# zhangrengang/SubPhaser

Measured on AMD Instinct MI355X. Metric: genome Gbases/s k-mer+enrichment, wheat k=15 1Mb windows, higher is better.
Workload: dtype u32

## Files before the change

### include/subphaser_hip.h

```cpp
#ifndef SUBPHASER_HIP_H
#define SUBPHASER_HIP_H
#include <stdint.h>
#ifdef __cplusplus
extern "C" {
#endif

#define SP_OK 0
#define SP_EINVAL (-1)
#define SP_EUNSUP (-2)
#define SP_ENOMEM (-3)
#define SP_EHIP (-4)
#define SP_ENODEV (-5)
#define SP_ESTATE (-6)
#define SP_EIO (-7)

typedef struct sp_ctx sp_ctx;

int sp_version(void);
const char *sp_last_error(const sp_ctx *ctx);

int sp_ctx_create(int device, void *stream, sp_ctx **out);
int sp_ctx_destroy(sp_ctx *ctx);
int sp_sync(sp_ctx *ctx);
void *sp_stream(sp_ctx *ctx);

int sp_genome_reset(sp_ctx *ctx, int n_chrom);
int sp_genome_add(sp_ctx *ctx, int chrom, const uint8_t *ascii, int64_t len);
int sp_genome_add_device(sp_ctx *ctx, int chrom, const uint8_t *d_ascii, int64_t len);
int sp_genome_len(sp_ctx *ctx, int chrom, int64_t *len);
int sp_genome_unpack(sp_ctx *ctx, int chrom, uint8_t *ascii_out, int64_t len);

int sp_count(sp_ctx *ctx, int k, int lower_count, int engine);
int sp_count_range(sp_ctx *ctx, int k, int lower_count, int engine, int first, int last);
int sp_count_recounts(sp_ctx *ctx, int64_t *recounts);
int sp_nslots(sp_ctx *ctx, int k, int64_t *nslots);
int sp_tables_bind(sp_ctx *ctx, int chrom, void *d_table);
int sp_table_overflow(sp_ctx *ctx, int chrom, void *d_pairs, int64_t cap, int64_t *n_pairs);
int sp_table_merge(sp_ctx *ctx, void *d_dst_u8, const void *d_dst_ovf, int64_t n_dst_ovf, const void *d_src_u8,
                   const void *d_src_ovf, int64_t n_src_ovf, int64_t slot_base, int64_t n, void *d_out_ovf, int64_t cap,
                   int64_t *n_out);
int sp_table_lengths(sp_ctx *ctx, const void *d_tab_u8, const void *d_ovf, int64_t n_ovf, int64_t slot_base, int64_t n,
                     int lower_count, int64_t *sum, int64_t *n_dump);
int sp_lengths(sp_ctx *ctx, int64_t *lengths );
int sp_dump_size(sp_ctx *ctx, int chrom, int64_t *n);
int sp_dump(sp_ctx *ctx, int chrom, uint64_t *keys, uint32_t *counts, int64_t cap, int64_t *n);

int sp_filter_view(sp_ctx *ctx, int C, const void *const *d_tabs, int64_t slot_base,
                   int64_t nslots_view, const int64_t *lengths, int k, int lower_count,
                   const void *const *d_ovf, const int64_t *n_ovf);
int sp_filter(sp_ctx *ctx, int n_sets, const int32_t *set_off, const int32_t *unit_off,
              const int32_t *unit_chrom, double min_fold, int baseline, double min_freq,
              double max_freq, double ratio, int64_t *n_union, int64_t *n_rows, int64_t *n_hist);
int sp_filter_fetch(sp_ctx *ctx, uint64_t *keys, uint32_t *counts, double *freqs, uint64_t *tot,
                    int64_t cap_rows);
int sp_filter_fetch_async(sp_ctx *ctx, uint64_t *keys, uint32_t *counts, uint64_t *tot, int64_t cap_rows);
int sp_filter_fetch_wait(sp_ctx *ctx);
int sp_filter_fetch_device(sp_ctx *ctx, void *d_keys, void *d_counts, void *d_tot, int64_t cap_rows);
int sp_filter_hist(sp_ctx *ctx, uint64_t *tot, int64_t cap);

int sp_labels_set(sp_ctx *ctx, const uint64_t *keys, const uint8_t *sg, int64_t n, int n_sg);
int sp_labels_set_device(sp_ctx *ctx, const uint64_t *d_keys, const uint8_t *d_sg, int64_t n, int n_sg);
int sp_map_nslots(sp_ctx *ctx, int chrom, int64_t bin_size, int64_t chunk_size, int64_t *nslots);
int sp_map_bins(sp_ctx *ctx, int chrom, int64_t bin_size, int64_t chunk_size, int32_t *slot_counts,
                int64_t nslots, int64_t *n_mapped);
int sp_map_bins_all(sp_ctx *ctx, int64_t bin_size, int64_t chunk_size, const int64_t *slot_off,
                    int32_t *slot_counts, int64_t *n_mapped);
int sp_stack_windows(sp_ctx *ctx, int64_t bin_size, int64_t chunk_size, int64_t window_size,
                     const int64_t *slot_off, const int64_t *win_off, int64_t *win_counts);
int sp_stack_windows_dev(sp_ctx *ctx, int64_t bin_size, int64_t chunk_size, int64_t window_size,
                         const int64_t *slot_off, const int64_t *win_off, const int64_t *seg_start, void *d_win);
int sp_map_features(sp_ctx *ctx, const uint8_t *ascii, const int64_t *off, int64_t n_feat,
                    int64_t *counts);
int sp_map_intervals(sp_ctx *ctx, const int32_t *chrom, const int64_t *start, const int64_t *end, int64_t n,
                     int64_t *counts);
int sp_labels_hit(sp_ctx *ctx, int64_t *n_hit);

int sp_enrich(sp_ctx *ctx, const int64_t *counts, int64_t W, int S, double max_pval,
              double min_ratio, double *pvals, int32_t *argmin, uint8_t *sig, double *ratios);
int sp_enrich_dev(sp_ctx *ctx, const void *d_counts, int64_t W, int S, double max_pval, double min_ratio,
                  double *pvals, int32_t *argmin, uint8_t *sig, double *ratios);
int sp_stack_enrich(sp_ctx *ctx, int64_t bin_size, int64_t chunk_size, int64_t window_size, const int64_t *slot_off,
                    const int64_t *win_off, double max_pval, double min_ratio, int64_t *win_counts, double *pvals,
                    int32_t *argmin, uint8_t *sig, double *ratios);

int sp_kmer_ttest(sp_ctx *ctx, const uint32_t *counts, int64_t M, int C, const int64_t *lengths, int n_groups,
                  const int32_t *group_off, const int32_t *group_chrom, int32_t *top, int32_t *second,
                  double *pvals, double *means);

int sp_sparse_sizes(sp_ctx *ctx, int64_t *n);
int sp_sparse_sample(sp_ctx *ctx, int chrom, int64_t n_samples, uint64_t *keys, int64_t *n_out);
int sp_sparse_split(sp_ctx *ctx, int chrom, const uint64_t *splitters, int n_split, int64_t *bounds);
int sp_sparse_export(sp_ctx *ctx, int chrom, int64_t first, int64_t count, void *d_keys, void *d_counts);
int sp_sparse_view(sp_ctx *ctx, int C, const void *const *d_keys, const void *const *d_counts, const int64_t *n,
                   const int64_t *lengths, int k, int lower_count);

int sp_prof_enable(sp_ctx *ctx, int on);
int sp_prof_reset(sp_ctx *ctx);
int sp_prof_report(sp_ctx *ctx, char *buf, int64_t cap);

int sp_synth_chrom(sp_ctx *ctx, uint8_t *d_out, int64_t len, uint64_t seed, int set_id,
                   int sg_id, int n_sg, int chrom_id, int exchange);
int sp_synth_chrom_range(sp_ctx *ctx, uint8_t *d_out, int64_t len, int64_t start, int64_t n, uint64_t seed, int set_id,
                         int sg_id, int n_sg, int chrom_id, int exchange);
int sp_host_alloc(sp_ctx *ctx, int64_t bytes, void **h_ptr);
int sp_host_free(sp_ctx *ctx, void *h_ptr);
int sp_host_register(sp_ctx *ctx, void *h_ptr, int64_t bytes);
int sp_host_unregister(sp_ctx *ctx, void *h_ptr);
int sp_dev_alloc(sp_ctx *ctx, int64_t bytes, void **d_ptr);
int sp_dev_free(sp_ctx *ctx, void *d_ptr);
int sp_dev_copy_to_host(sp_ctx *ctx, void *dst, const void *d_src, int64_t bytes);
int sp_dev_copy_from_host(sp_ctx *ctx, void *d_dst, const void *src, int64_t bytes);


typedef struct sp_fasta sp_fasta;
int sp_fasta_open(const void *data, int64_t n, int threads, sp_fasta **out);
int sp_fasta_counts(const sp_fasta *h, int64_t *n_records, int64_t *n_bases);
int sp_fasta_fetch(const sp_fasta *h, int64_t *hdr_start, int64_t *hdr_end, int64_t *seq_off, void *cat);
void sp_fasta_close(sp_fasta *h);


int sp_text_kmer_matrix(const uint64_t *keys, int k, const double *freqs, int64_t M, int C, int threads, int fd,
                        int64_t *bytes);
int sp_text_sig_kmers(const uint64_t *keys, int k, const int32_t *top, const char *names, int n_names,
                      const double *pvals, const double *means, int G, int64_t M, int threads, int fd, int64_t *bytes);
int sp_text_repr(const double *x, int64_t n, char *out, int64_t *off);

#define SP_COL_STR 0
#define SP_COL_I64 1
#define SP_COL_F64 2
#define SP_COL_NAME 3
#define SP_COL_IVAL 4
typedef struct sp_text_col {
    int kind;
    int width;
    char join;
    const void *data;
    const int64_t *off;
    const char *names;
} sp_text_col;
int sp_text_table(const sp_text_col *cols, int n_cols, int64_t M, int threads, int fd, int64_t *bytes);

#ifdef __cplusplus
}
#endif
#endif
```

### subphaser_amd/_native.py

```python
import ctypes as C
import json
import os

import numpy as np

_HERE = os.path.dirname(os.path.abspath(__file__))
LIB_PATH = os.environ.get("SUBPHASER_HIP_LIB") or os.path.join(_HERE, "lib", "libsubphaser_hip.so")

SP_OK, SP_EINVAL, SP_EUNSUP, SP_ENOMEM, SP_EHIP, SP_ENODEV, SP_ESTATE, SP_EIO = 0, -1, -2, -3, -4, -5, -6, -7

SYMBOLS = [
    "sp_version", "sp_last_error", "sp_ctx_create", "sp_ctx_destroy", "sp_sync", "sp_stream",
    "sp_genome_reset", "sp_genome_add", "sp_genome_add_device", "sp_genome_len", "sp_genome_unpack",
    "sp_count", "sp_count_range", "sp_count_recounts", "sp_nslots", "sp_tables_bind", "sp_table_overflow", "sp_table_merge", "sp_table_lengths", "sp_lengths", "sp_dump_size", "sp_dump",
    "sp_filter_view", "sp_filter", "sp_filter_fetch", "sp_filter_fetch_async", "sp_filter_fetch_wait", "sp_filter_fetch_device", "sp_filter_hist",
    "sp_labels_set", "sp_labels_set_device", "sp_map_nslots", "sp_map_bins", "sp_map_bins_all", "sp_stack_windows", "sp_stack_windows_dev", "sp_stack_enrich", "sp_map_features", "sp_map_intervals", "sp_labels_hit",
    "sp_enrich", "sp_enrich_dev", "sp_kmer_ttest",
    "sp_sparse_sizes", "sp_sparse_sample", "sp_sparse_split", "sp_sparse_export", "sp_sparse_view",
    "sp_prof_enable", "sp_prof_reset", "sp_prof_report",
    "sp_synth_chrom", "sp_synth_chrom_range", "sp_host_alloc", "sp_host_free", "sp_host_register", "sp_host_unregister", "sp_dev_alloc", "sp_dev_free", "sp_dev_copy_to_host", "sp_dev_copy_from_host",
    "sp_fasta_open", "sp_fasta_counts", "sp_fasta_fetch", "sp_fasta_close",
    "sp_text_kmer_matrix", "sp_text_sig_kmers", "sp_text_repr", "sp_text_table",
]


def csrc_fingerprint():
    import glob
    import hashlib
    h = hashlib.sha256()
    files = sorted(glob.glob(os.path.join(_HERE, "csrc", "*.hip")) + glob.glob(os.path.join(_HERE, "csrc", "*.h")))
    for f in files:
        h.update(os.path.basename(f).encode())
        h.update(open(f, "rb").read())
    return h.hexdigest()[:16]


class NativeError(RuntimeError):
    """HIP/runtime failure inside libsubphaser_hip.so."""


_lib = None


def load():
    global _lib
    if _lib is not None:
        return _lib
    if not os.path.exists(LIB_PATH):
        raise NativeError(
            "libsubphaser_hip.so is not built (%s). Run `python -c 'import __graft_entry__ as g; g.build()'` "
            "or `make -C subphaser_amd/csrc`. There is no CPU fallback." % LIB_PATH)
    L = C.CDLL(LIB_PATH)
    vp, i64, i32, dbl, ci = C.c_void_p, C.c_int64, C.c_int32, C.c_double, C.c_int
    P = C.POINTER
    L.sp_version.restype = ci
    L.sp_last_error.restype = C.c_char_p
    L.sp_last_error.argtypes = [vp]
    L.sp_ctx_create.argtypes = [ci, vp, P(vp)]
    L.sp_ctx_destroy.argtypes = [vp]
    L.sp_sync.argtypes = [vp]
    L.sp_stream.restype = vp
    L.sp_stream.argtypes = [vp]
    L.sp_genome_reset.argtypes = [vp, ci]
    L.sp_genome_add.argtypes = [vp, ci, vp, i64]
    L.sp_genome_add_device.argtypes = [vp, ci, vp, i64]
    L.sp_genome_len.argtypes = [vp, ci, P(i64)]
    L.sp_genome_unpack.argtypes = [vp, ci, vp, i64]
    L.sp_count.argtypes = [vp, ci, ci, ci]
    L.sp_count_range.argtypes = [vp, ci, ci, ci, ci, ci]
    L.sp_nslots.argtypes = [vp, ci, P(i64)]
    L.sp_count_recounts.argtypes = [vp, P(i64)]
    L.sp_tables_bind.argtypes = [vp, ci, vp]
    L.sp_table_overflow.argtypes = [vp, ci, vp, i64, P(i64)]
    L.sp_table_merge.argtypes = [vp, vp, vp, i64, vp, vp, i64, i64, i64, vp, i64, P(i64)]
    L.sp_table_lengths.argtypes = [vp, vp, vp, i64, i64, i64, ci, P(i64), P(i64)]
    L.sp_filter_view.argtypes = [vp, ci, vp, i64, i64, vp, ci, ci, vp, vp]
    L.sp_lengths.argtypes = [vp, vp]
    L.sp_dump_size.argtypes = [vp, ci, P(i64)]
    L.sp_dump.argtypes = [vp, ci, vp, vp, i64, P(i64)]
    L.sp_filter.argtypes = [vp, ci, vp, vp, vp, dbl, ci, dbl, dbl, dbl, P(i64), P(i64), P(i64)]
    L.sp_filter_fetch.argtypes = [vp, vp, vp, vp, vp, i64]
    L.sp_filter_fetch_device.argtypes = [vp, vp, vp, vp, i64]
    L.sp_filter_fetch_async.argtypes = [vp, vp, vp, vp, i64]
    L.sp_filter_fetch_wait.argtypes = [vp]
    L.sp_filter_hist.argtypes = [vp, vp, i64]
    L.sp_labels_set.argtypes = [vp, vp, vp, i64, ci]
    L.sp_labels_set_device.argtypes = [vp, vp, vp, i64, ci]
    L.sp_map_nslots.argtypes = [vp, ci, i64, i64, P(i64)]
    L.sp_map_bins.argtypes = [vp, ci, i64, i64, vp, i64, P(i64)]
    L.sp_map_bins_all.argtypes = [vp, i64, i64, vp, vp, vp]
    L.sp_stack_windows.argtypes = [vp, i64, i64, i64, vp, vp, vp]
    L.sp_stack_windows_dev.argtypes = [vp, i64, i64, i64, vp, vp, vp, vp]
    L.sp_stack_enrich.argtypes = [vp, i64, i64, i64, vp, vp, dbl, dbl, vp, vp, vp, vp, vp]
    L.sp_map_features.argtypes = [vp, vp, vp, i64, vp]
    L.sp_map_intervals.argtypes = [vp, vp, vp, vp, i64, vp]
    L.sp_host_alloc.argtypes = [vp, i64, P(vp)]
    L.sp_host_free.argtypes = [vp, vp]
    L.sp_labels_hit.argtypes = [vp, P(i64)]
    L.sp_enrich.argtypes = [vp, vp, i64, ci, dbl, dbl, vp, vp, vp, vp]
    L.sp_enrich_dev.argtypes = [vp, vp, i64, ci, dbl, dbl, vp, vp, vp, vp]
    L.sp_kmer_ttest.argtypes = [vp, vp, i64, ci, vp, ci, vp, vp, vp, vp, vp, vp]
    L.sp_sparse_sizes.argtypes = [vp, vp]
    L.sp_sparse_sample.argtypes = [vp, ci, i64, vp, P(i64)]
    L.sp_sparse_split.argtypes = [vp, ci, vp, ci, vp]
    L.sp_sparse_export.argtypes = [vp, ci, i64, i64, vp, vp]
    L.sp_sparse_view.argtypes = [vp, ci, vp, vp, vp, vp, ci, ci]
    L.sp_prof_enable.argtypes = [vp, ci]
    L.sp_prof_reset.argtypes = [vp]
    L.sp_prof_report.argtypes = [vp, C.c_char_p, i64]
    L.sp_synth_chrom.argtypes = [vp, vp, i64, C.c_uint64, ci, ci, ci, ci, ci]
    L.sp_synth_chrom_range.argtypes = [vp, vp, i64, i64, i64, C.c_uint64, ci, ci, ci, ci, ci]
    L.sp_dev_alloc.argtypes = [vp, i64, P(vp)]
    L.sp_dev_free.argtypes = [vp, vp]
    L.sp_dev_copy_to_host.argtypes = [vp, vp, vp, i64]
    L.sp_host_register.argtypes = [vp, vp, i64]
    L.sp_host_unregister.argtypes = [vp, vp]
    L.sp_dev_copy_from_host.argtypes = [vp, vp, vp, i64]
    L.sp_fasta_open.argtypes = [vp, i64, ci, P(vp)]
    L.sp_fasta_counts.argtypes = [vp, P(i64), P(i64)]
    L.sp_fasta_fetch.argtypes = [vp, vp, vp, vp, vp]
    L.sp_fasta_close.argtypes = [vp]
    L.sp_fasta_close.restype = None
    L.sp_text_kmer_matrix.argtypes = [vp, ci, vp, i64, ci, ci, ci, P(i64)]
    L.sp_text_sig_kmers.argtypes = [vp, ci, vp, C.c_char_p, ci, vp, vp, ci, i64, ci, ci, P(i64)]
    L.sp_text_repr.argtypes = [vp, i64, vp, vp]
    L.sp_text_table.argtypes = [vp, ci, i64, ci, ci, P(i64)]
    for name in SYMBOLS:
        if name not in ("sp_last_error", "sp_stream", "sp_fasta_close"):
            getattr(L, name).restype = ci
    _lib = L
    return L


def _p(a):
    return a.ctypes.data_as(C.c_void_p) if a is not None else None


def fasta_scan(data, threads=None, out=None):
    L = load()
    data = np.frombuffer(data, np.uint8) if isinstance(data, (bytes, bytearray, memoryview)) else data
    if data.dtype != np.uint8 or not data.flags.c_contiguous:
        data = np.ascontiguousarray(data, np.uint8)
    n = int(data.size)
    if threads is None:
        threads = min(32, len(os.sched_getaffinity(0)))
    h = C.c_void_p()
    rc = L.sp_fasta_open(C.c_void_p(data.ctypes.data) if n else None, n, int(threads), C.byref(h))
    if rc == SP_ENOMEM:
        raise MemoryError("sp_fasta_open")
    if rc:
        raise ValueError("sp_fasta_open: bad arguments")
    try:
        nr, nb = C.c_int64(), C.c_int64()
        L.sp_fasta_counts(h, C.byref(nr), C.byref(nb))
        nr, nb = nr.value, nb.value
        hs, he, off = np.empty(nr, np.int64), np.empty(nr, np.int64), np.empty(nr + 1, np.int64)
        cat = out(nb) if out is not None else np.empty(nb, np.uint8)
        if L.sp_fasta_fetch(h, _p(hs), _p(he), _p(off), _p(cat) if nb else None):
            raise ValueError("sp_fasta_fetch: bad arguments")
    finally:
        L.sp_fasta_close(h)
    ids = []
    for a, b in zip(hs.tolist(), he.tolist()):
        t = bytes(data[a:b]).split()
        ids.append(t[0].decode() if t else "")
    return ids, cat, off


def _fd_of(fout):
    try:
        fd = fout.fileno()
        fout.flush()
        return fd
    except Exception:
        return None


def _text_threads():
    return min(64, len(os.sched_getaffinity(0)))


def _text_fail(name, rc):
    msg = load().sp_last_error(None).decode(errors="replace")
    if rc == SP_ENOMEM:
        raise MemoryError("%s: %s" % (name, msg or "out of memory"))
    raise OSError("%s failed (%d): %s" % (name, rc, msg))


def text_kmer_matrix(fout, keys, k, freqs):
    fd = _fd_of(fout)
    if fd is None:
        return False
    keys = np.ascontiguousarray(keys, np.uint64)
    freqs = np.ascontiguousarray(freqs, np.float64)
    M, Cn = freqs.shape
    rc = load().sp_text_kmer_matrix(_p(keys), int(k), _p(freqs), M, Cn, _text_threads(), fd, None)
    if rc:
        _text_fail("sp_text_kmer_matrix", rc)
    return True


def text_sig_kmers(fout, keys, k, top, names, pvals, means):
    fd = _fd_of(fout)
    if fd is None:
        return False
    keys = np.ascontiguousarray(keys, np.uint64)
    top = np.ascontiguousarray(top, np.int32)
    pvals = np.ascontiguousarray(pvals, np.float64)
    means = np.ascontiguousarray(means, np.float64)
    blob = b"".join(n.encode() + b"\0" for n in names)
    rc = load().sp_text_sig_kmers(_p(keys), int(k), _p(top), blob, len(names), _p(pvals), _p(means), means.shape[1],
                                  len(keys), _text_threads(), fd, None)
    if rc:
        _text_fail("sp_text_sig_kmers", rc)
    return True


class _TextCol(C.Structure):
    _fields_ = [("kind", C.c_int), ("width", C.c_int), ("join", C.c_char), ("data", C.c_void_p),
                ("off", C.c_void_p), ("names", C.c_void_p)]


def str_blob(strings):
    enc = [s.encode() for s in strings]
    off = np.zeros(len(enc) + 1, np.int64)
    if enc:
        np.cumsum(np.fromiter((len(e) for e in enc), np.int64, len(enc)), out=off[1:])
    return np.frombuffer(b"".join(enc) or b"\0", np.uint8), off


def write_chunks(fout, n_rows, format_rows, chunk=50000):
    for lo in range(0, max(0, n_rows), chunk):
        fout.write(format_rows(lo, min(lo + chunk, n_rows)))


def text_table(fout, n_rows, cols):
    fd = _fd_of(fout)
    if fd is None:
        return False
    arr = (_TextCol * len(cols))()
    keep = []
    for c, col in zip(arr, cols):
        kind = col[0]
        if kind == "str":
            blob, off = np.ascontiguousarray(col[1], np.uint8), np.ascontiguousarray(col[2], np.int64)
            assert off.size == n_rows + 1
            c.kind, c.width, c.join, c.data, c.off = 0, 1, b"\t", blob.ctypes.data, off.ctypes.data
            keep += [blob, off]
        elif kind in ("i64", "f64"):
            a = np.ascontiguousarray(col[1], np.int64 if kind == "i64" else np.float64).reshape(n_rows, -1)
            c.kind, c.width, c.join, c.data = (1 if kind == "i64" else 2), max(1, a.shape[1]), col[2].encode(), a.ctypes.data
            keep.append(a)
        elif kind == "ival":
            a = np.ascontiguousarray(col[1], np.int64).reshape(n_rows, 3)
            blob, off = str_blob(col[2])
            c.kind, c.width, c.join, c.data, c.off, c.names = 4, len(col[2]), b"\t", a.ctypes.data, off.ctypes.data, blob.ctypes.data
            keep += [a, blob, off]
        elif kind == "name":
            idx = np.ascontiguousarray(col[1], np.int32)
            blob, off = str_blob(col[2])
            assert idx.size == n_rows
            c.kind, c.width, c.join, c.data, c.off, c.names = 3, len(col[2]), b"\t", idx.ctypes.data, off.ctypes.data, blob.ctypes.data
            keep += [idx, blob, off]
        else:
            raise ValueError(kind)
    rc = load().sp_text_table(arr, len(cols), int(n_rows), _text_threads(), fd, None)
    if rc:
        _text_fail("sp_text_table", rc)
    return True


def text_repr(x):
    x = np.ascontiguousarray(x, np.float64)
    out = np.empty(max(1, x.size * 40), np.uint8)
    off = np.empty(x.size + 1, np.int64)
    load().sp_text_repr(_p(x), x.size, _p(out), _p(off))
    b = out.tobytes()
    return [b[off[i]:off[i + 1]].decode() for i in range(x.size)]


def as_ascii(seq):
    if isinstance(seq, str):
        seq = seq.encode()
    if isinstance(seq, (bytes, bytearray, memoryview)):
        return np.frombuffer(seq, dtype=np.uint8)
    return np.ascontiguousarray(seq, dtype=np.uint8)


class Context:

    def __init__(self, device=0, stream=None):
        self.L = load()
        h = C.c_void_p()
        rc = self.L.sp_ctx_create(int(device), C.c_void_p(stream) if stream else None, C.byref(h))
        if rc != SP_OK:
            raise NativeError("sp_ctx_create failed (%d): %s" % (rc, self.L.sp_last_error(None).decode()))
        self.h = h
        self.n_chrom = 0
        self.k = None
        self._pinned = {}

    def _ck(self, rc):
        if rc == SP_OK:
            return
        msg = self.L.sp_last_error(self.h).decode()
        if rc in (SP_ESTATE, SP_EINVAL, SP_EUNSUP):
            raise ValueError(msg)
        if rc == SP_ENOMEM:
            raise MemoryError(msg)
        raise NativeError("libsubphaser_hip error %d: %s" % (rc, msg))

    def close(self):
        if getattr(self, "h", None):
            for d_keys, d_sg in getattr(self, "_label_copies", {}).values():
                self.L.sp_dev_free(self.h, C.c_void_p(d_keys))
                self.L.sp_dev_free(self.h, C.c_void_p(d_sg))
            self._label_copies = {}
            for ptr, _ in self._pinned.values():
                self.L.sp_host_free(self.h, C.c_void_p(ptr))
            self._pinned = {}
            self.L.sp_ctx_destroy(self.h)
            self.h = None

    def pinned_empty(self, tag, shape, dtype):
        dtype = np.dtype(dtype)
        n = int(np.prod(shape)) * dtype.itemsize
        ptr, cap = self._pinned.get(tag, (None, 0))
        if n > cap or ptr is None:
            if ptr:
                self.L.sp_host_free(self.h, C.c_void_p(ptr))
            p = C.c_void_p()
            want = n + n // 8 + 4096
            self._ck(self.L.sp_host_alloc(self.h, want, C.byref(p)))
            ptr, cap = p.value, want
            self._pinned[tag] = (ptr, cap)
        buf = (C.c_uint8 * max(n, 1)).from_address(ptr)
        return np.frombuffer(buf, dtype=dtype, count=int(np.prod(shape))).reshape(shape)

    def __del__(self):
        try:
            self.close()
        except Exception:
            pass

    def __enter__(self):
        return self

    def __exit__(self, *a):
        self.close()

    def sync(self):
        self._ck(self.L.sp_sync(self.h))

    @property
    def stream(self):
        return self.L.sp_stream(self.h)

    def genome_reset(self, n_chrom):
        self._ck(self.L.sp_genome_reset(self.h, int(n_chrom)))
        self.n_chrom = int(n_chrom)

    def genome_add(self, chrom, seq):
        a = as_ascii(seq)
        self._ck(self.L.sp_genome_add(self.h, int(chrom), _p(a), a.size))

    def genome_add_device(self, chrom, d_ptr, length):
        self._ck(self.L.sp_genome_add_device(self.h, int(chrom), C.c_void_p(int(d_ptr)), int(length)))

    def genome_len(self, chrom):
        n = C.c_int64()
        self._ck(self.L.sp_genome_len(self.h, int(chrom), C.byref(n)))
        return n.value

    def genome_unpack(self, chrom):
        n = self.genome_len(chrom)
        out = np.empty(n, np.uint8)
        self._ck(self.L.sp_genome_unpack(self.h, int(chrom), _p(out), n))
        return out

    def count(self, k, lower_count=3, engine=0):
        self._ck(self.L.sp_count(self.h, int(k), int(lower_count), int(engine)))
        self.k = int(k)

    def count_range(self, k, lower_count, engine, first, last):
        self._ck(self.L.sp_count_range(self.h, int(k), int(lower_count), int(engine), int(first), int(last)))
        self.k = int(k)

    def count_recounts(self):
        n = C.c_int64()
        self._ck(self.L.sp_count_recounts(self.h, C.byref(n)))
        return n.value

    def nslots(self, k):
        n = C.c_int64()
        self._ck(self.L.sp_nslots(self.h, int(k), C.byref(n)))
        return n.value

    def tables_bind(self, chrom, d_ptr):
        self._ck(self.L.sp_tables_bind(self.h, int(chrom), C.c_void_p(int(d_ptr)) if d_ptr else None))

    def table_overflow(self, chrom, d_pairs=None, cap=0):
        n = C.c_int64()
        self._ck(self.L.sp_table_overflow(self.h, int(chrom), C.c_void_p(int(d_pairs)) if d_pairs else None, int(cap),
                                          C.byref(n)))
        return n.value

    def table_merge(self, d_dst, d_dst_ovf, n_dst_ovf, d_src, d_src_ovf, n_src_ovf, slot_base, n, d_out_ovf, cap):
        m = C.c_int64()
        self._ck(self.L.sp_table_merge(self.h, C.c_void_p(int(d_dst)), C.c_void_p(int(d_dst_ovf)) if n_dst_ovf else None,
                                       int(n_dst_ovf), C.c_void_p(int(d_src)),
                                       C.c_void_p(int(d_src_ovf)) if n_src_ovf else None, int(n_src_ovf), int(slot_base),
                                       int(n), C.c_void_p(int(d_out_ovf)) if cap else None, int(cap), C.byref(m)))
        return m.value

    def table_lengths(self, d_tab, d_ovf, n_ovf, slot_base, n, lower_count):
        a, b = C.c_int64(), C.c_int64()
        self._ck(self.L.sp_table_lengths(self.h, C.c_void_p(int(d_tab)), C.c_void_p(int(d_ovf)) if n_ovf else None,
                                         int(n_ovf), int(slot_base), int(n), int(lower_count), C.byref(a), C.byref(b)))
        return a.value, b.value

    def filter_view(self, d_ptrs, slot_base, nslots_view, lengths, k, lower_count, d_ovf=None, n_ovf=None):
        if d_ptrs is None:
            self._ck(self.L.sp_filter_view(self.h, 0, None, 0, 0, None, 0, 0, None, None))
            self._view_C = None
            return
        arr = (C.c_void_p * len(d_ptrs))(*[int(p) for p in d_ptrs])
        lengths = np.ascontiguousarray(lengths, np.int64)
        oarr, narr = None, None
        if d_ovf is not None:
            oarr = (C.c_void_p * len(d_ptrs))(*[int(p) if p else None for p in d_ovf])
            narr = _p(np.ascontiguousarray(n_ovf, np.int64))
        self._ck(self.L.sp_filter_view(self.h, len(d_ptrs), arr, int(slot_base), int(nslots_view), _p(lengths),
                                       int(k), int(lower_count), oarr, narr))
        self._view_C = len(d_ptrs)
        self.k = int(k)

    def sparse_sizes(self):
        out = np.zeros(self.n_chrom, np.int64)
        if self.n_chrom:
            self._ck(self.L.sp_sparse_sizes(self.h, _p(out)))
        return out

    def sparse_sample(self, chrom, n_samples):
        out = np.empty(int(n_samples), np.uint64)
        n = C.c_int64()
        self._ck(self.L.sp_sparse_sample(self.h, int(chrom), int(n_samples), _p(out), C.byref(n)))
        return out[:n.value]

    def sparse_split(self, chrom, splitters):
        sp = np.ascontiguousarray(splitters, np.uint64)
        bounds = np.zeros(sp.size + 2, np.int64)
        self._ck(self.L.sp_sparse_split(self.h, int(chrom), _p(sp), int(sp.size), _p(bounds)))
        return bounds

    def sparse_export(self, chrom, first, count, d_keys, d_counts):
        v = lambda p: C.c_void_p(int(p)) if p else None
        self._ck(self.L.sp_sparse_export(self.h, int(chrom), int(first), int(count), v(d_keys), v(d_counts)))

    def sparse_view(self, d_keys, d_counts, n, lengths, k, lower_count):
        if d_keys is None:
            self._ck(self.L.sp_sparse_view(self.h, 0, None, None, None, None, 0, 0))
            self._view_C = None
            return
        ka = (C.c_void_p * len(d_keys))(*[int(p) for p in d_keys])
        ca = (C.c_void_p * len(d_counts))(*[int(p) for p in d_counts])
        n = np.ascontiguousarray(n, np.int64)
        lengths = np.ascontiguousarray(lengths, np.int64)
        self._ck(self.L.sp_sparse_view(self.h, len(d_keys), ka, ca, _p(n), _p(lengths), int(k), int(lower_count)))
        self._view_C = len(d_keys)
        self.k = int(k)

    def lengths(self):
        out = np.zeros(self.n_chrom, np.int64)
        self._ck(self.L.sp_lengths(self.h, _p(out)))
        return out

    def dump_size(self, chrom):
        n = C.c_int64()
        self._ck(self.L.sp_dump_size(self.h, int(chrom), C.byref(n)))
        return n.value

    def dump(self, chrom, sort=True):
        n = C.c_int64()
        self._ck(self.L.sp_dump_size(self.h, int(chrom), C.byref(n)))
        keys = np.empty(n.value, np.uint64)
        cnts = np.empty(n.value, np.uint32)
        self._ck(self.L.sp_dump(self.h, int(chrom), _p(keys), _p(cnts), n.value, C.byref(n)))
        if sort and keys.size:
            o = np.argsort(keys, kind="stable")
            keys, cnts = keys[o], cnts[o]
        return keys, cnts

    def filter(self, set_off, unit_off, unit_chrom, min_fold, baseline, min_freq, max_freq, ratio):
        set_off = np.ascontiguousarray(set_off, np.int32)
        unit_off = np.ascontiguousarray(unit_off, np.int32)
        unit_chrom = np.ascontiguousarray(unit_chrom, np.int32)
        nu, nr, nh = C.c_int64(), C.c_int64(), C.c_int64()
        self._ck(self.L.sp_filter(self.h, len(set_off) - 1, _p(set_off), _p(unit_off), _p(unit_chrom),
                                  float(min_fold), int(baseline), float(min_freq), float(max_freq),
                                  float(ratio), C.byref(nu), C.byref(nr), C.byref(nh)))
        return nu.value, nr.value, nh.value

    def filter_fetch(self, n_rows, want_freqs=True, sort=True, pinned=False):
        Cn = getattr(self, "_view_C", None) or self.n_chrom
        if pinned and not sort:
            keys = self.pinned_empty("ff_keys", (n_rows,), np.uint64)
            counts = self.pinned_empty("ff_counts", (n_rows, Cn), np.uint32)
            tot = self.pinned_empty("ff_tot", (n_rows,), np.uint64)
            freqs = self.pinned_empty("ff_freqs", (n_rows, Cn), np.float64) if want_freqs else None
        else:
            keys = np.empty(n_rows, np.uint64)
            counts = np.empty((n_rows, Cn), np.uint32)
            tot = np.empty(n_rows, np.uint64)
            freqs = np.empty((n_rows, Cn), np.float64) if want_freqs else None
        self._ck(self.L.sp_filter_fetch(self.h, _p(keys), _p(counts), _p(freqs), _p(tot), n_rows))
        if sort and n_rows:
            o = np.argsort(keys, kind="stable")
            keys, counts, tot = keys[o], counts[o], tot[o]
            if freqs is not None:
                freqs = freqs[o]
        return keys, counts, freqs, tot

    def filter_fetch_async(self, n_rows):
        Cn = getattr(self, "_view_C", None) or self.n_chrom
        keys = self.pinned_empty("ff_keys", (n_rows,), np.uint64)
        counts = self.pinned_empty("ff_counts", (n_rows, Cn), np.uint32)
        tot = self.pinned_empty("ff_tot", (n_rows,), np.uint64)
        self._ck(self.L.sp_filter_fetch_async(self.h, _p(keys), _p(counts), _p(tot), n_rows))
        return keys, counts, tot

    def filter_fetch_async_ptr(self, h_keys, h_counts, n_rows):
        tot = self.pinned_empty("ff_tot", (max(int(n_rows), 1),), np.uint64)
        self._ck(self.L.sp_filter_fetch_async(self.h, C.c_void_p(int(h_keys)), C.c_void_p(int(h_counts)), _p(tot), int(n_rows)))

    def filter_fetch_wait(self):
        self._ck(self.L.sp_filter_fetch_wait(self.h))

    def filter_fetch_device(self, d_keys, d_counts, d_tot, n_rows):
        v = lambda p: C.c_void_p(int(p)) if p else None
        self._ck(self.L.sp_filter_fetch_device(self.h, v(d_keys), v(d_counts), v(d_tot), int(n_rows)))

    def filter_hist(self, n_hist):
        tot = np.empty(n_hist, np.uint64)
        self._ck(self.L.sp_filter_hist(self.h, _p(tot), n_hist))
        return tot

    def labels_set(self, keys, sg, n_sg):
        keys = np.ascontiguousarray(keys, np.uint64)
        sg = np.ascontiguousarray(sg, np.uint8)
        assert keys.size == sg.size
        self._ck(self.L.sp_labels_set(self.h, _p(keys), _p(sg), keys.size, int(n_sg)))
        self.n_sg = int(n_sg)

    def labels_set_device(self, d_keys, d_sg, n, n_sg):
        self._ck(self.L.sp_labels_set_device(self.h, C.c_void_p(int(d_keys)), C.c_void_p(int(d_sg)), int(n), int(n_sg)))
        self.n_sg = int(n_sg)

    def labels_set_from(self, labels, n_sg):
        if hasattr(labels, "on_device"):
            d_keys, d_sg = labels.on_device(self)
            self.labels_set_device(d_keys, d_sg, len(labels.keys), n_sg)
        else:
            self.labels_set(labels.keys, labels.sg_idx, n_sg)

    def map_nslots(self, chrom, bin_size, chunk_size):
        n = C.c_int64()
        self._ck(self.L.sp_map_nslots(self.h, int(chrom), int(bin_size), int(chunk_size), C.byref(n)))
        return n.value

    def map_bins(self, chrom, bin_size=10000, chunk_size=10_000_000):
        ns = self.map_nslots(chrom, bin_size, chunk_size)
        out = np.empty((ns, self.n_sg), np.int32)
        n = C.c_int64()
        self._ck(self.L.sp_map_bins(self.h, int(chrom), int(bin_size), int(chunk_size), _p(out), ns,
                                    C.byref(n)))
        return out, n.value

    def map_bins_all(self, bin_size=10000, chunk_size=10_000_000):
        off = np.zeros(self.n_chrom + 1, np.int64)
        for i in range(self.n_chrom):
            off[i + 1] = off[i] + self.map_nslots(i, bin_size, chunk_size)
        out = self.pinned_empty("map_all", (int(off[-1]), self.n_sg), np.int32)
        nm = np.zeros(self.n_chrom, np.int64)
        self._ck(self.L.sp_map_bins_all(self.h, int(bin_size), int(chunk_size), _p(off), _p(out), _p(nm)))
        self.last_map = (out, off)
        return [out[off[i]:off[i + 1]] for i in range(self.n_chrom)], nm

    def stack_windows(self, bin_size, chunk_size, window_size, lengths):
        out, off = self.last_map
        woff = np.zeros(self.n_chrom + 1, np.int64)
        for i, n in enumerate(lengths):
            woff[i + 1] = woff[i] + (int(n) + int(window_size) - 1) // int(window_size) + 1
        win = self.pinned_empty("win_all", (int(woff[-1]), self.n_sg), np.int64)
        self._ck(self.L.sp_stack_windows(self.h, int(bin_size), int(chunk_size), int(window_size), _p(off),
                                         _p(woff), _p(win)))
        return win, woff

    def stack_windows_dev(self, bin_size, chunk_size, window_size, win_off, seg_start, d_win):
        out, off = self.last_map
        win_off = np.ascontiguousarray(win_off, np.int64)
        seg = np.ascontiguousarray(seg_start, np.int64) if seg_start is not None else None
        self._ck(self.L.sp_stack_windows_dev(self.h, int(bin_size), int(chunk_size), int(window_size), _p(off),
                                             _p(win_off), _p(seg) if seg is not None else None, C.c_void_p(int(d_win))))

    def stack_enrich(self, bin_size, chunk_size, window_size, lengths, max_pval=0.05, min_ratio=0.5):
        out, off = self.last_map
        woff = np.zeros(self.n_chrom + 1, np.int64)
        for i, n in enumerate(lengths):
            woff[i + 1] = woff[i] + (int(n) + int(window_size) - 1) // int(window_size) + 1
        W, S = int(woff[-1]), self.n_sg
        win = self.pinned_empty("win_all", (W, S), np.int64)
        pvals = self.pinned_empty("enr_p", (W, S), np.float64)
        ratios = self.pinned_empty("enr_q", (W, S), np.float64)
        argmin = self.pinned_empty("enr_a", (W,), np.int32)
        sig = self.pinned_empty("enr_s", (W,), np.uint8)
        self._ck(self.L.sp_stack_enrich(self.h, int(bin_size), int(chunk_size), int(window_size), _p(off), _p(woff),
                                        float(max_pval), float(min_ratio), _p(win), _p(pvals), _p(argmin), _p(sig),
                                        _p(ratios)))
        return win, woff, pvals, argmin, sig, ratios

    def enrich_dev(self, d_counts, W, S, max_pval=0.05, min_ratio=0.5):
        pvals = np.empty((W, S), np.float64)
        ratios = np.empty((W, S), np.float64)
        argmin = np.empty(W, np.int32)
        sig = np.empty(W, np.uint8)
        self._ck(self.L.sp_enrich_dev(self.h, C.c_void_p(int(d_counts)), int(W), int(S), float(max_pval),
                                      float(min_ratio), _p(pvals), _p(argmin), _p(sig), _p(ratios)))
        return pvals, argmin, sig.astype(bool), ratios

    def map_features(self, seqs):
        arrs = [as_ascii(s) for s in seqs]
        off = np.zeros(len(arrs) + 1, np.int64)
        for i, a in enumerate(arrs):
            off[i + 1] = off[i] + a.size
        cat = np.concatenate(arrs) if arrs else np.empty(0, np.uint8)
        cat = np.ascontiguousarray(cat)
        out = np.zeros((len(arrs), self.n_sg), np.int64)
        self._ck(self.L.sp_map_features(self.h, _p(cat), _p(off), len(arrs), _p(out)))
        return out

    def map_features_cat(self, cat, off):
        cat = np.ascontiguousarray(cat, np.uint8)
        off = np.ascontiguousarray(off, np.int64)
        n = off.size - 1
        out = np.zeros((n, self.n_sg), np.int64)
        self._ck(self.L.sp_map_features(self.h, _p(cat), _p(off), n, _p(out)))
        return out

    def map_intervals(self, chrom, start, end):
        chrom = np.ascontiguousarray(chrom, np.int32)
        start = np.ascontiguousarray(start, np.int64)
        end = np.ascontiguousarray(end, np.int64)
        assert chrom.size == start.size == end.size
        out = np.zeros((chrom.size, self.n_sg), np.int64)
        self._ck(self.L.sp_map_intervals(self.h, _p(chrom), _p(start), _p(end), chrom.size, _p(out)))
        return out

    def labels_hit(self):
        n = C.c_int64()
        self._ck(self.L.sp_labels_hit(self.h, C.byref(n)))
        return n.value

    def enrich(self, counts, max_pval=0.05, min_ratio=0.5):
        counts = np.ascontiguousarray(counts, np.int64)
        if counts.ndim != 2:
            raise ValueError("counts must be W x S")
        W, S = counts.shape
        pvals = np.empty((W, S), np.float64)
        ratios = np.empty((W, S), np.float64)
        argmin = np.empty(W, np.int32)
        sig = np.empty(W, np.uint8)
        self._ck(self.L.sp_enrich(self.h, _p(counts), W, S, float(max_pval), float(min_ratio), _p(pvals),
                                  _p(argmin), _p(sig), _p(ratios)))
        return pvals, argmin, sig.astype(bool), ratios

    def kmer_ttest(self, counts, lengths, groups):
        if isinstance(counts, tuple):
            d_ptr, M, Cn = counts
            cptr = C.c_void_p(int(d_ptr))
        else:
            counts = np.ascontiguousarray(counts, np.uint32)
            M, Cn = counts.shape
            cptr = _p(counts)
        lengths = np.ascontiguousarray(lengths, np.int64)
        goff = np.zeros(len(groups) + 1, np.int32)
        goff[1:] = np.cumsum([len(g) for g in groups])
        gch = np.ascontiguousarray(np.concatenate([np.asarray(g, np.int32) for g in groups]), np.int32)
        top, second = np.empty(M, np.int32), np.empty(M, np.int32)
        pvals, means = np.empty(M, np.float64), np.empty((M, len(groups)), np.float64)
        self._ck(self.L.sp_kmer_ttest(self.h, cptr, M, Cn, _p(lengths), len(groups), _p(goff), _p(gch),
                                      _p(top), _p(second), _p(pvals), _p(means)))
        return top, second, pvals, means

    def stage_rows(self, counts):
        counts = np.ascontiguousarray(counts, np.uint32)
        old = getattr(self, "_staged_rows", None)
        if old:
            self.dev_free(old)
            self._staged_rows = None
        if counts.size == 0:
            return None
        self._staged_rows = self.dev_alloc(counts.nbytes)
        self.host_to_dev(self._staged_rows, counts)
        return (self._staged_rows, counts.shape[0], counts.shape[1])

    def release_rows(self):
        old = getattr(self, "_staged_rows", None)
        if old:
            self.dev_free(old)
            self._staged_rows = None

    def prof_enable(self, on=True):
        self._ck(self.L.sp_prof_enable(self.h, 1 if on else 0))

    def prof_reset(self):
        self._ck(self.L.sp_prof_reset(self.h))

    def prof_report(self):
        buf = C.create_string_buffer(1 << 16)
        self._ck(self.L.sp_prof_report(self.h, buf, len(buf)))
        return json.loads(buf.value.decode())

    def dev_alloc(self, nbytes):
        p = C.c_void_p()
        self._ck(self.L.sp_dev_alloc(self.h, int(nbytes), C.byref(p)))
        return p.value

    def dev_free(self, ptr):
        self._ck(self.L.sp_dev_free(self.h, C.c_void_p(ptr)))

    def dev_to_host(self, ptr, nbytes, offset=0):
        out = np.empty(nbytes, np.uint8)
        self._ck(self.L.sp_dev_copy_to_host(self.h, _p(out), C.c_void_p(ptr + offset), int(nbytes)))
        return out

    def host_register(self, h_ptr, nbytes):
        self._ck(self.L.sp_host_register(self.h, C.c_void_p(int(h_ptr)), int(nbytes)))

    def host_unregister(self, h_ptr):
        self._ck(self.L.sp_host_unregister(self.h, C.c_void_p(int(h_ptr))))

    def dev_to_host_ptr(self, h_ptr, d_ptr, nbytes):
        if nbytes:
            self._ck(self.L.sp_dev_copy_to_host(self.h, C.c_void_p(int(h_ptr)), C.c_void_p(int(d_ptr)), int(nbytes)))

    def host_to_dev(self, ptr, arr, offset=0):
        arr = np.ascontiguousarray(arr)
        self._ck(self.L.sp_dev_copy_from_host(self.h, C.c_void_p(ptr + offset), _p(arr), int(arr.nbytes)))

    def synth_chrom_range(self, d_ptr, length, start, n, seed, set_id, sg_id, n_sg, chrom_id, exchange=0):
        self._ck(self.L.sp_synth_chrom_range(self.h, C.c_void_p(d_ptr), int(length), int(start), int(n), int(seed),
                                             int(set_id), int(sg_id), int(n_sg), int(chrom_id), int(exchange)))

    def synth_chrom(self, d_ptr, length, seed, set_id, sg_id, n_sg, chrom_id, exchange=0):
        self._ck(self.L.sp_synth_chrom(self.h, C.c_void_p(d_ptr), int(length), int(seed), int(set_id),
                                       int(sg_id), int(n_sg), int(chrom_id), int(exchange)))
```

### subphaser_amd/csrc/sp_common.h

```cpp
#pragma once
#include <hip/hip_runtime.h>
#include <stdint.h>
#include <stdio.h>
#include <string.h>

#include <map>
#include <string>
#include <vector>

#include "../../include/subphaser_hip.h"

#define SP_WAVE 64

struct sp_chrom {
    bool tab_external = false;
    int64_t len = 0;
    int64_t nw = 0;
    int64_t cap_mw = 0;
    uint32_t *d_pk = nullptr;
    uint32_t *d_pm = nullptr;
    uint32_t *d_nm = nullptr;
    uint8_t *d_tab = nullptr;
    uint2 *d_ovf = nullptr;
    int64_t n_ovf = 0, cap_ovf = 0;
    uint32_t *d_ovf_idx = nullptr;
    int64_t ovf_idx_n = 0, ovf_idx_cap = 0;
    int64_t length_sum = 0;
    int64_t n_dump = 0;
    hipEvent_t ev_packed = nullptr;
};
#define SP_PAD_WORDS 8
#define SP_LIST_MAXC 1024
#define SP_TABLE_LDS (140 * 1024)
#define SP_TABLE_MIN_TILE 256
#define SP_TABLE_MAXC (SP_TABLE_LDS / SP_TABLE_MIN_TILE)
#ifndef SP_DERIVE_PM
#define SP_DERIVE_PM 1
#endif

struct sp_buf {
    void *p = nullptr;
    int64_t cap = 0;
};

template <typename T>
struct sp_tmp {
    T *p = nullptr;
    sp_tmp() = default;
    sp_tmp(const sp_tmp &) = delete;
    sp_tmp &operator=(const sp_tmp &) = delete;
    ~sp_tmp() {
        if (p) hipFree(p);
    }
    hipError_t alloc(size_t n_elems) { return hipMalloc((void **)&p, (n_elems ? n_elems : 1) * sizeof(T)); }
    operator T *() const { return p; }
};

struct sp_sparse_chrom {
    uint64_t *d_keys = nullptr;
    uint32_t *d_cnts = nullptr;
    int64_t n = 0, cap = 0, length_sum = 0;
};

struct sp_tabref {
    const uint8_t *tab;
    const uint2 *ovf;
    int64_t n_ovf;
    const uint32_t *ovf_idx = nullptr;
};

struct sp_prof_entry {
    std::string name;
    hipEvent_t e0, e1;
};

struct sp_ctx {
    int device = 0;
    hipStream_t stream = nullptr;
    hipStream_t copy_stream = nullptr;
    hipEvent_t copy_event = nullptr;
    bool own_stream = false;
    int n_cu = 256;
    std::string err;
    std::vector<sp_chrom> chroms;
    int k = 0;
    int lower = 0;
    int64_t nslots = 0;
    bool counted = false;
    int64_t c2_recounts = 0;
    bool fv_on = false;
    std::vector<sp_tabref> fv_tabs;
    std::vector<int64_t> fv_lengths;
    int64_t fv_slot_base = 0, fv_nslots = 0;
    bool sv_on = false;
    std::vector<const uint64_t *> sv_keys;
    std::vector<const uint32_t *> sv_cnts;
    std::vector<int64_t> sv_n;
    bool filtered = false;
    int64_t n_union = 0, n_rows = 0, n_hist = 0;
    uint32_t *d_flag_row = nullptr;
    uint32_t *d_flag_hist = nullptr;
    uint64_t *d_blk_row = nullptr;
    uint64_t *d_blk_hist = nullptr;
    int64_t n_fblocks = 0;
    uint8_t *d_label = nullptr;
    sp_buf b_ptab, b_labkeys;
    int ptab_k = 0;
    int64_t ptab_n = 0;
    unsigned long long *h_lflags = nullptr;
    sp_buf b_lflags;
    int64_t bloom_last_n = -1;
    int bloom_last_bits = 0, bloom_last_k = 0;
    sp_buf b_ctab, b_covf;
    int ct_bb = 0;
    uint32_t ct_ovf_mask = 0;
    int sq_bb = 0;
    uint64_t sq_ovf_mask = 0;
    int map_engine = 0;
    bool labels_ready = false;
    uint32_t *d_bloom = nullptr;
    int bloom_bits = 0;
    int n_sg = 0;
    int64_t n_labels = 0;
    void *d_scratch = nullptr;
    int64_t scratch_bytes = 0;
    void *d_ws2 = nullptr;
    int64_t ws2_bytes = 0;
    sp_buf b_cntlen;
    sp_buf b_tab32, b_ovfw;
    struct lane_t {
        hipStream_t stream = nullptr;
        hipEvent_t done = nullptr;
        void *d_ws2 = nullptr;
        int64_t ws2_bytes = 0;
        sp_buf b_ovfw;
        void *h_desc = nullptr;
        int64_t h_desc_cap = 0;
        sp_buf b_sp_a, b_sp_b, b_sp_c, b_sp_tmp, b_s3_small;
        hipEvent_t ev_a = nullptr, ev_b = nullptr;
    };
#define SP_MAX_LANES 7
    lane_t lanes[SP_MAX_LANES];
    lane_t *lane = nullptr;
    void *h_desc = nullptr;
    int64_t h_desc_cap = 0;
    hipEvent_t lane_go = nullptr;
    bool sparse_mode = false;
    bool list_mode = false;
    std::vector<sp_sparse_chrom> sparse;
    sp_buf b_sp_a, b_sp_b, b_sp_c, b_sp_tmp, b_sf_keys, b_sf_counts, b_sf_tot, b_sf_hist, b_s3_small, b_slots;
    unsigned long long *h_s3 = nullptr;
    hipEvent_t s3_ev[2] = {nullptr, nullptr};
    int64_t sf_n = 0;
    uint64_t *d_hkeys = nullptr;
    int64_t hcap = 0;
    sp_buf b_tt;
    sp_buf b_wtab, b_enr;
    sp_buf b_fq;
    sp_buf b_fflat;
    sp_buf b_map, b_mapdesc, b_ival, b_emit, b_fpar, b_win;
    bool map_all_valid = false;
    bool prof = false;
    std::vector<sp_prof_entry> prof_pending;
    std::map<std::string, std::pair<int64_t, double>> prof_acc;
};

extern thread_local std::string g_sp_err;

int sp_fail(sp_ctx *ctx, int code, const char *fmt, ...);
int sp_scratch(sp_ctx *ctx, int64_t bytes, void **out);
struct sp_ctx;
int sp_buf_ensure(sp_ctx *ctx, sp_buf &b, int64_t bytes);
void sp_buf_free(sp_buf &b);
void sp_prof_begin(sp_ctx *ctx, const char *name);
void sp_prof_end(sp_ctx *ctx);
void sp_prof_flush(sp_ctx *ctx);

#define SP_HIP(ctx, call)                                                                  \
    do {                                                                                   \
        hipError_t e__ = (call);                                                           \
        if (e__ != hipSuccess)                                                             \
            return sp_fail(ctx, e__ == hipErrorOutOfMemory ? SP_ENOMEM : SP_EHIP,          \
                           "%s failed: %s (%s:%d)", #call, hipGetErrorString(e__), __FILE__, \
                           __LINE__);                                                      \
    } while (0)

#define SP_LAUNCH(ctx, name, kernel, grid, block, shmem, ...)                       \
    do {                                                                            \
        sp_prof_begin(ctx, name);                                                   \
        hipLaunchKernelGGL(kernel, grid, block, shmem, (ctx)->stream, __VA_ARGS__); \
        sp_prof_end(ctx);                                                           \
        SP_HIP(ctx, hipGetLastError());                                             \
    } while (0)

struct sp_kparams {
    int k;
    int odd;
    uint64_t kmask;
    int rcshift;
};

__host__ __device__ inline sp_kparams sp_make_kparams(int k) {
    sp_kparams p;
    p.k = k;
    p.odd = k & 1;
    p.kmask = (k == 32) ? ~0ULL : ((1ULL << (2 * k)) - 1ULL);
    p.rcshift = 2 * (k - 1);
    return p;
}

__host__ __device__ inline int64_t sp_dense_slots(int k) {
    return (k & 1) ? (1LL << (2 * k - 1)) : (1LL << (2 * k));
}

__host__ __device__ inline uint64_t sp_slot_of(uint64_t fwd, uint64_t rc, const sp_kparams &p) {
    if (p.odd) {
        uint64_t rep = ((fwd >> p.k) & 1ULL) ? rc : fwd;
        uint64_t lowmask = (1ULL << p.k) - 1ULL;
        return (rep & lowmask) | ((rep >> (p.k + 1)) << p.k);
    }
    return fwd < rc ? fwd : rc;
}

__host__ __device__ inline uint64_t sp_revcomp(uint64_t x, int k) {
    x = ~x;
    x = ((x >> 2) & 0x3333333333333333ULL) | ((x & 0x3333333333333333ULL) << 2);
    x = ((x >> 4) & 0x0F0F0F0F0F0F0F0FULL) | ((x & 0x0F0F0F0F0F0F0F0FULL) << 4);
    x = ((x >> 8) & 0x00FF00FF00FF00FFULL) | ((x & 0x00FF00FF00FF00FFULL) << 8);
    x = ((x >> 16) & 0x0000FFFF0000FFFFULL) | ((x & 0x0000FFFF0000FFFFULL) << 16);
    x = (x >> 32) | (x << 32);
    return x >> (64 - 2 * k);
}

__host__ __device__ inline uint64_t sp_key_of_slot(uint64_t slot, const sp_kparams &p) {
    if (p.odd) {
        uint64_t lowmask = (1ULL << p.k) - 1ULL;
        uint64_t rep = (slot & lowmask) | ((slot >> p.k) << (p.k + 1));
        uint64_t r = sp_revcomp(rep, p.k);
        return rep < r ? rep : r;
    }
    return slot;
}

__host__ __device__ inline uint64_t sp_slot_of_key(uint64_t key, const sp_kparams &p) {
    return sp_slot_of(key, sp_revcomp(key, p.k), p);
}
```

### subphaser_amd/csrc/sp_ctx.hip

```cpp
#include <stdarg.h>

#include "sp_common.h"

thread_local std::string g_sp_err;

int sp_fail(sp_ctx *ctx, int code, const char *fmt, ...) {
    char buf[1024];
    va_list ap;
    va_start(ap, fmt);
    vsnprintf(buf, sizeof buf, fmt, ap);
    va_end(ap);
    if (ctx) ctx->err = buf;
    g_sp_err = buf;
    return code;
}

int sp_scratch(sp_ctx *ctx, int64_t bytes, void **out) {
    if (bytes > ctx->scratch_bytes) {
        if (ctx->d_scratch) {
            SP_HIP(ctx, hipStreamSynchronize(ctx->stream));
            SP_HIP(ctx, hipFree(ctx->d_scratch));
            ctx->d_scratch = nullptr;
            ctx->scratch_bytes = 0;
        }
        SP_HIP(ctx, hipMalloc(&ctx->d_scratch, (size_t)bytes));
        ctx->scratch_bytes = bytes;
    }
    *out = ctx->d_scratch;
    return SP_OK;
}

int sp_buf_ensure(sp_ctx *ctx, sp_buf &b, int64_t bytes) {
    if (bytes <= b.cap) return SP_OK;
    if (b.p) {
        SP_HIP(ctx, hipStreamSynchronize(ctx->stream));
        SP_HIP(ctx, hipFree(b.p));
        b.p = nullptr;
        b.cap = 0;
    }
    int64_t want = bytes + bytes / 8 + 4096;
    SP_HIP(ctx, hipMalloc(&b.p, (size_t)want));
    b.cap = want;
    return SP_OK;
}
void sp_buf_free(sp_buf &b) {
    if (b.p) hipFree(b.p);
    b.p = nullptr;
    b.cap = 0;
}

void sp_prof_begin(sp_ctx *ctx, const char *name) {
    if (!ctx->prof) return;
    sp_prof_entry e;
    e.name = name;
    hipEventCreate(&e.e0);
    hipEventCreate(&e.e1);
    hipEventRecord(e.e0, ctx->stream);
    ctx->prof_pending.push_back(e);
}
void sp_prof_end(sp_ctx *ctx) {
    if (!ctx->prof) return;
    hipEventRecord(ctx->prof_pending.back().e1, ctx->stream);
}
void sp_prof_flush(sp_ctx *ctx) {
    if (ctx->prof_pending.empty()) return;
    hipStreamSynchronize(ctx->stream);
    for (auto &e : ctx->prof_pending) {
        float ms = 0.f;
        hipEventElapsedTime(&ms, e.e0, e.e1);
        auto &acc = ctx->prof_acc[e.name];
        acc.first += 1;
        acc.second += ms;
        hipEventDestroy(e.e0);
        hipEventDestroy(e.e1);
    }
    ctx->prof_pending.clear();
}

void sp_sparse_release(sp_ctx *ctx);

extern "C" {

int sp_version(void) { return 100; }

const char *sp_last_error(const sp_ctx *ctx) { return ctx ? ctx->err.c_str() : g_sp_err.c_str(); }

int sp_ctx_create(int device, void *stream, sp_ctx **out) {
    if (!out) return sp_fail(nullptr, SP_EINVAL, "sp_ctx_create: out is NULL");
    int n = 0;
    if (hipGetDeviceCount(&n) != hipSuccess || n <= 0)
        return sp_fail(nullptr, SP_ENODEV, "no HIP device visible (libsubphaser_hip needs an MI355X)");
    if (device < 0 || device >= n)
        return sp_fail(nullptr, SP_EINVAL, "device %d out of range (0..%d)", device, n - 1);
    sp_ctx *ctx = new sp_ctx();
    ctx->device = device;
    SP_HIP(ctx, hipSetDevice(device));
    hipDeviceProp_t prop;
    SP_HIP(ctx, hipGetDeviceProperties(&prop, device));
    ctx->n_cu = prop.multiProcessorCount;
    if (stream) {
        ctx->stream = (hipStream_t)stream;
    } else {
        SP_HIP(ctx, hipStreamCreateWithFlags(&ctx->stream, hipStreamNonBlocking));
        ctx->own_stream = true;
    }
    *out = ctx;
    return SP_OK;
}

static void free_chrom(sp_chrom &c) {
    if (c.d_pk) hipFree(c.d_pk);
    if (c.d_nm) hipFree(c.d_nm);
    if (c.d_tab && !c.tab_external) hipFree(c.d_tab);
    if (c.d_ovf) hipFree(c.d_ovf);
    if (c.d_ovf_idx) hipFree(c.d_ovf_idx);
    c.d_ovf_idx = nullptr;
    c.ovf_idx_n = c.ovf_idx_cap = 0;
    if (c.ev_packed) hipEventDestroy(c.ev_packed);
    c = sp_chrom();
}

static void free_filter(sp_ctx *ctx) {
    if (ctx->d_flag_row) hipFree(ctx->d_flag_row);
    if (ctx->d_flag_hist) hipFree(ctx->d_flag_hist);
    if (ctx->d_blk_row) hipFree(ctx->d_blk_row);
    if (ctx->d_blk_hist) hipFree(ctx->d_blk_hist);
    ctx->d_flag_row = ctx->d_flag_hist = nullptr;
    ctx->d_blk_row = ctx->d_blk_hist = nullptr;
    ctx->filtered = false;
}

int sp_ctx_destroy(sp_ctx *ctx) {
    if (!ctx) return SP_OK;
    hipSetDevice(ctx->device);
    hipStreamSynchronize(ctx->stream);
    sp_prof_flush(ctx);
    for (auto &c : ctx->chroms) free_chrom(c);
    free_filter(ctx);
    sp_sparse_release(ctx);
    if (ctx->d_label) hipFree(ctx->d_label);
    if (ctx->d_bloom) hipFree(ctx->d_bloom);
    if (ctx->d_scratch) hipFree(ctx->d_scratch);
    if (ctx->d_ws2) hipFree(ctx->d_ws2);
    for (auto &ln : ctx->lanes) {
        if (ln.d_ws2) hipFree(ln.d_ws2);
        sp_buf_free(ln.b_ovfw);
        if (ln.h_desc) hipHostFree(ln.h_desc);
        sp_buf_free(ln.b_sp_a);
        sp_buf_free(ln.b_sp_b);
        sp_buf_free(ln.b_sp_c);
        sp_buf_free(ln.b_sp_tmp);
        sp_buf_free(ln.b_s3_small);
        if (ln.ev_a) hipEventDestroy(ln.ev_a);
        if (ln.ev_b) hipEventDestroy(ln.ev_b);
        if (ln.done) hipEventDestroy(ln.done);
        if (ln.stream) hipStreamDestroy(ln.stream);
    }
    if (ctx->lane_go) hipEventDestroy(ctx->lane_go);
    if (ctx->h_s3) hipHostFree(ctx->h_s3);
    if (ctx->h_desc) hipHostFree(ctx->h_desc);
    for (auto &e : ctx->s3_ev)
        if (e) hipEventDestroy(e);
    sp_buf_free(ctx->b_map);
    sp_buf_free(ctx->b_mapdesc);
    sp_buf_free(ctx->b_ival);
    sp_buf_free(ctx->b_ptab);
    sp_buf_free(ctx->b_lflags);
    if (ctx->h_lflags) hipHostFree(ctx->h_lflags);
    sp_buf_free(ctx->b_cntlen);
    sp_buf_free(ctx->b_ctab);
    sp_buf_free(ctx->b_covf);
    sp_buf_free(ctx->b_tab32);
    sp_buf_free(ctx->b_ovfw);
    sp_buf_free(ctx->b_labkeys);
    sp_buf_free(ctx->b_emit);
    sp_buf_free(ctx->b_slots);
    sp_buf_free(ctx->b_fpar);
    sp_buf_free(ctx->b_fflat);
    sp_buf_free(ctx->b_fq);
    sp_buf_free(ctx->b_wtab);
    sp_buf_free(ctx->b_enr);
    sp_buf_free(ctx->b_tt);
    sp_buf_free(ctx->b_win);
    if (ctx->copy_stream) {
        hipStreamSynchronize(ctx->copy_stream);
        hipStreamDestroy(ctx->copy_stream);
        hipEventDestroy(ctx->copy_event);
    }
    if (ctx->own_stream) hipStreamDestroy(ctx->stream);
    delete ctx;
    return SP_OK;
}

int sp_sync(sp_ctx *ctx) {
    SP_HIP(ctx, hipStreamSynchronize(ctx->stream));
    return SP_OK;
}

void *sp_stream(sp_ctx *ctx) { return (void *)ctx->stream; }

int sp_genome_reset(sp_ctx *ctx, int n_chrom) {
    if (!ctx || n_chrom < 0) return sp_fail(ctx, SP_EINVAL, "sp_genome_reset: bad arguments");
    SP_HIP(ctx, hipSetDevice(ctx->device));
    SP_HIP(ctx, hipStreamSynchronize(ctx->stream));
    if ((size_t)n_chrom == ctx->chroms.size()) {
        for (auto &c : ctx->chroms) {
            c.len = 0;
            c.nw = 0;
            c.length_sum = 0;
            c.n_dump = 0;
            c.n_ovf = 0;
            c.ovf_idx_n = 0;
        }
    } else {
        for (auto &c : ctx->chroms) free_chrom(c);
        ctx->chroms.assign((size_t)n_chrom, sp_chrom());
    }
    ctx->counted = false;
    ctx->filtered = false;
    return SP_OK;
}
}

__device__ __forceinline__ void pack_byte(uint32_t b, uint32_t &code, uint32_t &inv) {
    uint32_t u = b & 0xDFu;
    code = ((b >> 1) ^ (b >> 2)) & 3u;
    inv = !(u == 'A' || u == 'C' || u == 'G' || u == 'T');
}

__device__ __forceinline__ void pack_word4(uint32_t w, uint32_t &c8, uint32_t &inv4) {
    uint32_t t = ((w >> 1) ^ (w >> 2)) & 0x03030303u;
    const uint32_t letters = __builtin_amdgcn_perm(0u, 0x54474341u, t);
    const uint32_t x = letters ^ (w & 0xDFDFDFDFu);
    const uint32_t f = ((((x & 0x7F7F7F7Fu) + 0x7F7F7F7Fu) | x) & 0x80808080u) >> 7;
    t &= ~(f * 3u);
    t |= t >> 6;
    t |= t >> 12;
    c8 = t & 0xFFu;
    inv4 = ((f * 0x00204081u) >> 21) & 0xFu;
}
__device__ __forceinline__ uint32_t pack_msb_first(uint32_t w) {
    const uint32_t r = __brev(w);
    return ((r & 0x55555555u) << 1) | ((r >> 1) & 0x55555555u);
}

__global__ void __launch_bounds__(256)
k0_pack(const uint8_t *__restrict__ ascii, int64_t len, uint32_t *__restrict__ pk, uint32_t *__restrict__ pm,
        uint32_t *__restrict__ nm, int64_t n_mask_words) {
    int64_t t = (int64_t)blockIdx.x * blockDim.x + threadIdx.x;
    int64_t stride = (int64_t)gridDim.x * blockDim.x;
    const bool aligned = (((uintptr_t)ascii) & 15) == 0;
    for (; t < n_mask_words; t += stride) {
        int64_t base = t * 32;
        uint32_t w0 = 0, w1 = 0, m = 0, r0 = 0, r1 = 0;
        if (base + 32 <= len && aligned) {
            const uint4 *p = reinterpret_cast<const uint4 *>(ascii + base);
            uint4 a = p[0], b = p[1];
            uint32_t v[8] = {a.x, a.y, a.z, a.w, b.x, b.y, b.z, b.w};
#pragma unroll
            for (int q = 0; q < 8; q++) {
                uint32_t c8, inv4;
                pack_word4(v[q], c8, inv4);
                if (q < 4) w0 |= c8 << (8 * q);
                else w1 |= c8 << (8 * (q - 4));
                m |= inv4 << (4 * q);
            }
            r0 = pack_msb_first(w0);
            r1 = pack_msb_first(w1);
        } else {
            for (int i = 0; i < 32; i++) {
                uint32_t c = 0, iv = 1;
                if (base + i < len) pack_byte(ascii[base + i], c, iv);
                if (iv) c = 0;
                if (i < 16) { w0 |= c << (2 * i); r0 |= c << (30 - 2 * i); }
                else { w1 |= c << (2 * (i - 16)); r1 |= c << (30 - 2 * (i - 16)); }
                m |= iv << i;
            }
        }
        *reinterpret_cast<uint2 *>(pk + 2 * t) = make_uint2(w0, w1);
#if !SP_DERIVE_PM
        *reinterpret_cast<uint2 *>(pm + 2 * t) = make_uint2(r0, r1);
#else
        (void)r0; (void)r1; (void)pm;
#endif
        nm[t] = m;
    }
}

__global__ void __launch_bounds__(256)
k0_unpack(const uint32_t *__restrict__ pk, const uint32_t *__restrict__ nm, int64_t len,
          uint8_t *__restrict__ out) {
    int64_t i = (int64_t)blockIdx.x * blockDim.x + threadIdx.x;
    int64_t stride = (int64_t)gridDim.x * blockDim.x;
    for (; i < len; i += stride) {
        uint32_t c = (pk[i >> 4] >> (2 * (i & 15))) & 3u;
        uint32_t iv = (nm[i >> 5] >> (i & 31)) & 1u;
        out[i] = iv ? 'N' : "ACGT"[c];
    }
}

static int genome_add_impl(sp_ctx *ctx, int chrom, const uint8_t *d_ascii, int64_t len) {
    sp_chrom &c = ctx->chroms[(size_t)chrom];
    c.len = len;
    c.length_sum = 0;
    c.n_dump = 0;
    int64_t nmw = (len + 31) / 32 + SP_PAD_WORDS;
    c.nw = (len + 15) / 16;
    if (nmw > c.cap_mw) {
        if (c.d_pk) hipFree(c.d_pk);
        if (c.d_nm) hipFree(c.d_nm);
        c.d_pk = c.d_pm = c.d_nm = nullptr;
        c.cap_mw = 0;
#if SP_DERIVE_PM
        SP_HIP(ctx, hipMalloc(&c.d_pk, (size_t)(2 * nmw) * sizeof(uint32_t)));
        c.d_pm = c.d_pk;
#else
        SP_HIP(ctx, hipMalloc(&c.d_pk, (size_t)(4 * nmw) * sizeof(uint32_t)));
        c.d_pm = c.d_pk + 2 * nmw;
#endif
        SP_HIP(ctx, hipMalloc(&c.d_nm, (size_t)nmw * sizeof(uint32_t)));
        c.cap_mw = nmw;
    }
    int64_t blocks = (nmw + 255) / 256;
    if (blocks > 8LL * ctx->n_cu * 8) blocks = 8LL * ctx->n_cu * 8;
    if (blocks < 1) blocks = 1;
    SP_LAUNCH(ctx, "k0_pack", k0_pack, dim3((unsigned)blocks), dim3(256), 0, d_ascii, len, c.d_pk,
              c.d_pm, c.d_nm, nmw);
    if (!c.ev_packed) SP_HIP(ctx, hipEventCreateWithFlags(&c.ev_packed, hipEventDisableTiming));
    SP_HIP(ctx, hipEventRecord(c.ev_packed, ctx->stream));
    ctx->counted = false;
    return SP_OK;
}

extern "C" {

int sp_genome_add_device(sp_ctx *ctx, int chrom, const uint8_t *d_ascii, int64_t len) {
    if (!ctx || chrom < 0 || chrom >= (int)ctx->chroms.size() || len < 0 || (!d_ascii && len > 0))
        return sp_fail(ctx, SP_EINVAL, "sp_genome_add_device: bad arguments (chrom=%d len=%lld)", chrom,
                       (long long)len);
    SP_HIP(ctx, hipSetDevice(ctx->device));
    return genome_add_impl(ctx, chrom, d_ascii, len);
}

int sp_genome_add(sp_ctx *ctx, int chrom, const uint8_t *ascii, int64_t len) {
    if (!ctx || chrom < 0 || chrom >= (int)ctx->chroms.size() || len < 0 || (!ascii && len > 0))
        return sp_fail(ctx, SP_EINVAL, "sp_genome_add: bad arguments (chrom=%d len=%lld)", chrom,
                       (long long)len);
    SP_HIP(ctx, hipSetDevice(ctx->device));
    uint8_t *d = nullptr;
    SP_HIP(ctx, hipMalloc(&d, (size_t)(len > 0 ? len : 1)));
    hipError_t e = hipMemcpyAsync(d, ascii, (size_t)len, hipMemcpyHostToDevice, ctx->stream);
    int rc = SP_OK;
    if (e != hipSuccess) rc = sp_fail(ctx, SP_EHIP, "H2D copy failed: %s", hipGetErrorString(e));
    if (rc == SP_OK) rc = genome_add_impl(ctx, chrom, d, len);
    hipStreamSynchronize(ctx->stream);
    hipFree(d);
    return rc;
}

int sp_genome_len(sp_ctx *ctx, int chrom, int64_t *len) {
    if (!ctx || !len || chrom < 0 || chrom >= (int)ctx->chroms.size())
        return sp_fail(ctx, SP_EINVAL, "sp_genome_len: bad arguments");
    *len = ctx->chroms[(size_t)chrom].len;
    return SP_OK;
}

int sp_genome_unpack(sp_ctx *ctx, int chrom, uint8_t *ascii_out, int64_t len) {
    if (!ctx || chrom < 0 || chrom >= (int)ctx->chroms.size() || !ascii_out)
        return sp_fail(ctx, SP_EINVAL, "sp_genome_unpack: bad arguments");
    sp_chrom &c = ctx->chroms[(size_t)chrom];
    if (len != c.len) return sp_fail(ctx, SP_EINVAL, "sp_genome_unpack: len mismatch");
    if (len == 0) return SP_OK;
    SP_HIP(ctx, hipSetDevice(ctx->device));
    uint8_t *d = nullptr;
    SP_HIP(ctx, hipMalloc(&d, (size_t)len));
    int64_t blocks = (len + 255) / 256;
    if (blocks > 65536) blocks = 65536;
    SP_LAUNCH(ctx, "k0_unpack", k0_unpack, dim3((unsigned)blocks), dim3(256), 0, c.d_pk, c.d_nm, len, d);
    SP_HIP(ctx, hipMemcpyAsync(ascii_out, d, (size_t)len, hipMemcpyDeviceToHost, ctx->stream));
    SP_HIP(ctx, hipStreamSynchronize(ctx->stream));
    hipFree(d);
    return SP_OK;
}

int sp_prof_enable(sp_ctx *ctx, int on) {
    if (!ctx) return SP_EINVAL;
    if (!on) sp_prof_flush(ctx);
    ctx->prof = on != 0;
    return SP_OK;
}
int sp_prof_reset(sp_ctx *ctx) {
    if (!ctx) return SP_EINVAL;
    sp_prof_flush(ctx);
    ctx->prof_acc.clear();
    return SP_OK;
}
int sp_prof_report(sp_ctx *ctx, char *buf, int64_t cap) {
    if (!ctx || !buf || cap < 3) return SP_EINVAL;
    sp_prof_flush(ctx);
    std::string s = "{";
    bool first = true;
    for (auto &kv : ctx->prof_acc) {
        char tmp[256];
        snprintf(tmp, sizeof tmp, "%s\"%s\": {\"calls\": %lld, \"ms\": %.6f}", first ? "" : ", ",
                 kv.first.c_str(), (long long)kv.second.first, kv.second.second);
        s += tmp;
        first = false;
    }
    s += "}";
    if ((int64_t)s.size() + 1 > cap) return sp_fail(ctx, SP_EINVAL, "sp_prof_report: buffer too small");
    memcpy(buf, s.c_str(), s.size() + 1);
    return SP_OK;
}

int sp_host_alloc(sp_ctx *ctx, int64_t bytes, void **h_ptr) {
    if (!ctx || !h_ptr || bytes < 0) return sp_fail(ctx, SP_EINVAL, "sp_host_alloc: bad arguments");
    SP_HIP(ctx, hipSetDevice(ctx->device));
    SP_HIP(ctx, hipHostMalloc(h_ptr, (size_t)(bytes > 0 ? bytes : 1), hipHostMallocDefault));
    return SP_OK;
}
int sp_host_free(sp_ctx *ctx, void *h_ptr) {
    if (!ctx) return SP_EINVAL;
    SP_HIP(ctx, hipHostFree(h_ptr));
    return SP_OK;
}
int sp_host_register(sp_ctx *ctx, void *h_ptr, int64_t bytes) {
    if (!ctx || !h_ptr || bytes <= 0) return sp_fail(ctx, SP_EINVAL, "sp_host_register: bad arguments");
    SP_HIP(ctx, hipSetDevice(ctx->device));
    SP_HIP(ctx, hipHostRegister(h_ptr, (size_t)bytes, hipHostRegisterPortable));
    return SP_OK;
}
int sp_host_unregister(sp_ctx *ctx, void *h_ptr) {
    if (!ctx || !h_ptr) return SP_EINVAL;
    SP_HIP(ctx, hipHostUnregister(h_ptr));
    return SP_OK;
}
int sp_dev_alloc(sp_ctx *ctx, int64_t bytes, void **d_ptr) {
    if (!ctx || !d_ptr || bytes < 0) return sp_fail(ctx, SP_EINVAL, "sp_dev_alloc: bad arguments");
    SP_HIP(ctx, hipSetDevice(ctx->device));
    SP_HIP(ctx, hipMalloc(d_ptr, (size_t)(bytes > 0 ? bytes : 1)));
    return SP_OK;
}
int sp_dev_free(sp_ctx *ctx, void *d_ptr) {
    if (!ctx) return SP_EINVAL;
    SP_HIP(ctx, hipStreamSynchronize(ctx->stream));
    SP_HIP(ctx, hipFree(d_ptr));
    return SP_OK;
}
int sp_dev_copy_to_host(sp_ctx *ctx, void *dst, const void *d_src, int64_t bytes) {
    if (!ctx || !dst || !d_src || bytes < 0) return sp_fail(ctx, SP_EINVAL, "sp_dev_copy_to_host: bad arguments");
    SP_HIP(ctx, hipMemcpyAsync(dst, d_src, (size_t)bytes, hipMemcpyDeviceToHost, ctx->stream));
    SP_HIP(ctx, hipStreamSynchronize(ctx->stream));
    return SP_OK;
}
int sp_dev_copy_from_host(sp_ctx *ctx, void *d_dst, const void *src, int64_t bytes) {
    if (!ctx || !d_dst || !src || bytes < 0) return sp_fail(ctx, SP_EINVAL, "sp_dev_copy_from_host: bad arguments");
    SP_HIP(ctx, hipMemcpyAsync(d_dst, src, (size_t)bytes, hipMemcpyHostToDevice, ctx->stream));
    SP_HIP(ctx, hipStreamSynchronize(ctx->stream));
    return SP_OK;
}
}
```

### subphaser_amd/csrc/sp_filter.hip

```cpp
#include "sp_device.h"
#include "sp_filter.h"

#ifndef F_BLOCK
#define F_BLOCK 256
#endif
#ifndef F_GROUPS_PER_WAVE
#define F_GROUPS_PER_WAVE 64
#endif
#define F_WAVES (F_BLOCK / 64)
#define F_SLOTS_PER_BLOCK (F_WAVES * F_GROUPS_PER_WAVE * 64)
#ifndef F_TILE_BYTES
#define F_TILE_BYTES (24 * 1024)
#endif

#define F3_CHROM_MASK 0xfffff
#define F3_UNIT_END (1 << 20)
#define F3_SET_END (1 << 21)
#define F3_TOT (1 << 22)
#define F3_BI1 (1 << 23)

struct sp_filter_params {
    int C;
    int n_sets;
    int baseline;
    uint32_t lower;
    double min_fold, min_freq, max_freq, ratio;
    int64_t nslots;
    int64_t slot_base;
    int TS;
    int n_multi;
    int need_active;
    int need_hist;
    int fast;
    int R, R_sets;
    const int32_t *rowdesc;
    const float *rowinv;
    const int32_t *row_of_chrom;
    uint32_t *gq;
    unsigned long long *gq_n;
    unsigned long long gq_cap;
};

__device__ __forceinline__ uint32_t k3_ge_mask(uint32_t x, uint32_t addL ) {
    return (((x & 0x7f7f7f7fu) + addL) | x) & 0x80808080u;
}

#ifndef K3_STAGE
#define K3_STAGE 6
#endif
#ifndef K3_SCAN_CH
#define K3_SCAN_CH 4
#endif
#ifndef K3_WALK_CH
#define K3_WALK_CH 8
#endif
template <bool SWAR, int NCH>
__global__ void __launch_bounds__(F_BLOCK)
k3_eval(const sp_tabref *__restrict__ tabs, sp_filter_params P,
        const int32_t *__restrict__ set_off, const int32_t *__restrict__ unit_off,
        const int32_t *__restrict__ unit_chrom, const double *__restrict__ unit_den,
        unsigned long long *__restrict__ bm_row, unsigned long long *__restrict__ bm_hist,
        unsigned long long *__restrict__ blk_row, unsigned long long *__restrict__ blk_hist,
        unsigned long long *__restrict__ n_union) {
    extern __shared__ __attribute__((aligned(16))) uint8_t tile[];
    __shared__ unsigned long long red[16];
    __shared__ uint32_t s_qn, s_q2n, s_q3n;
    __shared__ unsigned long long s_gq0;
    const int TS = P.TS, R = P.R;
    const int32_t *__restrict__ rowdesc = P.rowdesc;
    const float *__restrict__ rowinv = P.rowinv;
    uint16_t *queue = reinterpret_cast<uint16_t *>(tile + (size_t)R * TS), *queue2 = queue + TS;
    uint32_t *bmr = reinterpret_cast<uint32_t *>(queue2 + TS), *bmh = bmr + TS / 32;
    const uint2 **l_ovf = reinterpret_cast<const uint2 **>(bmh + TS / 32);
    unsigned long long *l_novf = reinterpret_cast<unsigned long long *>(l_ovf + R);
    uint32_t *resolved = reinterpret_cast<uint32_t *>(l_novf + R);
    for (int r = threadIdx.x; r < R; r += F_BLOCK) {
        const int c = rowdesc[r] & F3_CHROM_MASK;
        l_ovf[r] = tabs[c].ovf;
        l_novf[r] = (unsigned long long)tabs[c].n_ovf;
    }
    uint32_t mk_unit = 0, mk_set = 0, mk_bi1 = 0, mk_tot = 0;
    int inv_bits = 0;
    if (NCH > 0) {
        const int d = rowdesc[threadIdx.x & 31];
        const unsigned long long b_unit = __ballot((d & F3_UNIT_END) != 0), b_set = __ballot((d & F3_SET_END) != 0);
        const unsigned long long b_bi1 = __ballot((d & F3_BI1) != 0), b_tot = __ballot((d & F3_TOT) != 0);
        mk_unit = (uint32_t)b_unit; mk_set = (uint32_t)b_set; mk_bi1 = (uint32_t)b_bi1; mk_tot = (uint32_t)b_tot;
        inv_bits = __float_as_int(rowinv[threadIdx.x & 31]);
    }
    mk_unit = __builtin_amdgcn_readfirstlane(mk_unit);
    mk_set = __builtin_amdgcn_readfirstlane(mk_set);
    mk_bi1 = __builtin_amdgcn_readfirstlane(mk_bi1);
    mk_tot = __builtin_amdgcn_readfirstlane(mk_tot);
    const int lane = threadIdx.x & 63;
    unsigned long long nrow = 0, nhist = 0, nuni = 0;
    const int64_t blk_base = (int64_t)blockIdx.x * F_SLOTS_PER_BLOCK;
    const uint32_t addL = (0x80u - P.lower) * 0x01010101u;
    const float fold32 = (float)P.min_fold;
    sp_fsets F;
    F.n_sets = P.n_sets;
    F.n_multi = P.n_multi;
    F.baseline = P.baseline;
    F.set_off = set_off;
    F.unit_off = unit_off;
    F.unit_chrom = unit_chrom;
    F.unit_den = unit_den;
    F.unit_inv = unit_den + set_off[P.n_sets];
    F.min_fold = P.min_fold;
    F.min_freq = P.min_freq;
    F.max_freq = P.max_freq;
    F.ratio = P.ratio;
    for (int64_t base = blk_base; base < blk_base + F_SLOTS_PER_BLOCK && base < P.nslots; base += TS) {
        const int n16 = TS / 16, total16 = R * n16;
        if (threadIdx.x == 0) s_qn = s_q2n = 0;
        for (int i = threadIdx.x; i < TS / 16; i += F_BLOCK) reinterpret_cast<uint32_t *>(bmr)[i] = 0;
        const bool whole = base + TS <= P.nslots && (n16 & 63) == 0;
        if (whole)
        for (int i0 = threadIdx.x; i0 < total16; i0 += K3_STAGE * F_BLOCK) {
            uint32_t vx[K3_STAGE], vy[K3_STAGE], vz[K3_STAGE], vw[K3_STAGE];
#pragma unroll
            for (int q = 0; q < K3_STAGE; q++) {
                int iw = __builtin_amdgcn_readfirstlane(i0 - lane + q * F_BLOCK);
                iw = iw < total16 ? iw : total16 - 64;
                const int r = iw / n16, j0 = iw - r * n16;
                const uint8_t *__restrict__ tab = tabs[rowdesc[r] & F3_CHROM_MASK].tab;
                const uint4 t = *reinterpret_cast<const uint4 *>(tab + base + (int64_t)(j0 + lane) * 16);
                vx[q] = t.x; vy[q] = t.y; vz[q] = t.z; vw[q] = t.w;
            }
#pragma unroll
            for (int q = 0; q < K3_STAGE; q++) {
                const int i = i0 + q * F_BLOCK;
                if (i < total16) reinterpret_cast<uint4 *>(tile)[i] = make_uint4(vx[q], vy[q], vz[q], vw[q]);
            }
        }
        if (!whole)
        for (int i0 = threadIdx.x; i0 < total16; i0 += 8 * F_BLOCK) {
            uint4 v[8];
#pragma unroll
            for (int q = 0; q < 8; q++) {
                const int i = i0 + q * F_BLOCK;
                v[q] = make_uint4(0, 0, 0, 0);
                if (i < total16) {
                    const int r = i / n16, j = i - r * n16;
                    const uint8_t *__restrict__ tab = tabs[rowdesc[r] & F3_CHROM_MASK].tab;
                    const int64_t s0 = base + (int64_t)j * 16;
                    if (s0 + 16 <= P.nslots) {
                        v[q] = *reinterpret_cast<const uint4 *>(tab + s0);
                    } else if (s0 < P.nslots) {
                        uint32_t w0 = 0, w1 = 0, w2 = 0, w3 = 0;
                        for (int b = 0; b < 16 && s0 + b < P.nslots; b++) {
                            const uint32_t y = (uint32_t)tab[s0 + b] << (8 * (b & 3));
                            if (b < 4) w0 |= y; else if (b < 8) w1 |= y; else if (b < 12) w2 |= y; else w3 |= y;
                        }
                        v[q] = make_uint4(w0, w1, w2, w3);
                    }
                }
            }
#pragma unroll
            for (int q = 0; q < 8; q++) {
                const int i = i0 + q * F_BLOCK;
                if (i < total16) reinterpret_cast<uint4 *>(tile)[i] = v[q];
            }
        }
        __syncthreads();
        const uint32_t *tw = reinterpret_cast<const uint32_t *>(tile);
        const int nw = TS / 4;
        for (int g = threadIdx.x; g < nw; g += F_BLOCK) {
            uint32_t any = 0, is255 = 0, qual;
            if (SWAR) {
                uint32_t act = 0, m = 0;
                if (NCH > 0) {
                    const uint32_t *col = tw + g;
                    for (int r0 = 0; r0 < R; r0 += K3_SCAN_CH) {
                        uint32_t x[K3_SCAN_CH];
#pragma unroll
                        for (int i = 0; i < K3_SCAN_CH; i++) x[i] = col[(r0 + i < R ? r0 + i : R - 1) * nw];
#pragma unroll
                        for (int i = 0; i < K3_SCAN_CH; i++) {
                            if (r0 + i < R) {
                                const uint32_t lo = x[i] & 0x7f7f7f7fu;
                                m |= (lo + addL) | x[i];
                                is255 |= (lo + 0x01010101u) & x[i];
                                if ((mk_set >> (r0 + i)) & 1u) {
                                    asm volatile("");
                                    m &= 0x80808080u;
                                    any |= m;
                                    act += m >> 7;
                                    m = 0;
                                }
                            }
                        }
                    }
                    any |= m & 0x80808080u;
                } else {
                    for (int r = 0; r < R; r++) {
                        const uint32_t x = tw[r * nw + g];
                        const uint32_t ge = k3_ge_mask(x, addL);
                        any |= ge;
                        is255 |= ((x & 0x7f7f7f7fu) + 0x01010101u) & x;
                        m |= ge;
                        if (rowdesc[r] & F3_SET_END) {
                            act += m >> 7;
                            m = 0;
                        }
                    }
                }
                is255 &= 0x80808080u;
                nuni += __popc(any);
                qual = P.need_active > 0 ? any & k3_ge_mask(act, (0x80u - (uint32_t)P.need_active) * 0x01010101u) : any;
            } else {
                for (int r = 0; r < R; r++) {
                    const uint32_t x = tw[r * nw + g];
#pragma unroll
                    for (int b = 0; b < 4; b++) {
                        const uint32_t y = (x >> (8 * b)) & 255u;
                        if (y == 255u) is255 |= 0x80u << (8 * b);
                        if (y == 255u || y >= P.lower) any |= 0x80u << (8 * b);
                    }
                }
                qual = any;
            }
            const uint32_t slow = (SWAR && NCH > 0 && P.fast) ? is255 : 0x80808080u;
            const uint32_t q_fast = qual & ~slow & 0x80808080u, q_slow = qual & slow & 0x80808080u;
            {
                unsigned long long bal[4];
                uint32_t n = 0;
#pragma unroll
                for (int b = 0; b < 4; b++) {
                    bal[b] = __ballot((q_fast >> (8 * b + 7)) & 1u);
                    n += (uint32_t)__popcll(bal[b]);
                }
                if (n) {
                    uint32_t qb = 0;
                    if (lane == 0) qb = atomicAdd(&s_qn, n);
                    qb = (uint32_t)__builtin_amdgcn_readfirstlane((int)qb);
#pragma unroll
                    for (int b = 0; b < 4; b++) {
                        if ((q_fast >> (8 * b + 7)) & 1u)
                            queue[qb + __builtin_amdgcn_mbcnt_hi((uint32_t)(bal[b] >> 32), __builtin_amdgcn_mbcnt_lo((uint32_t)bal[b], 0u))] = (uint16_t)(4 * g + b);
                        qb += (uint32_t)__popcll(bal[b]);
                    }
                }
            }
            if (__ballot(q_slow != 0u)) {
                unsigned long long bal[4];
                uint32_t n = 0;
#pragma unroll
                for (int b = 0; b < 4; b++) {
                    bal[b] = __ballot((q_slow >> (8 * b + 7)) & 1u);
                    n += (uint32_t)__popcll(bal[b]);
                }
                uint32_t qb = 0;
                if (lane == 0) qb = atomicAdd(&s_q2n, n);
                qb = (uint32_t)__builtin_amdgcn_readfirstlane((int)qb);
#pragma unroll
                for (int b = 0; b < 4; b++) {
                    if ((q_slow >> (8 * b + 7)) & 1u)
                        queue2[qb + __builtin_amdgcn_mbcnt_hi((uint32_t)(bal[b] >> 32), __builtin_amdgcn_mbcnt_lo((uint32_t)bal[b], 0u))] = (uint16_t)(4 * g + b);
                    qb += (uint32_t)__popcll(bal[b]);
                }
            }
        }
        __syncthreads();
        if (NCH > 0) {
            const uint32_t qn = s_qn;
            for (uint32_t q0 = 0; q0 < qn; q0 += F_BLOCK) {
                if ((uint32_t)__builtin_amdgcn_readfirstlane((int)(q0 + (threadIdx.x & ~63u))) >= qn) continue;
                const uint32_t q = q0 + threadIdx.x;
                const bool live = q < qn;
                const int sl = live ? (int)queue[q] : 0;
                int include = 0;
                bool exact = false;
                uint32_t tot = 0, num = 0;
                float m1 = -1.0f, m2 = -1.0f, mn = 3e38f;
                for (int r0 = 0; r0 < R; r0 += K3_WALK_CH) {
                    uint32_t y[K3_WALK_CH];
#pragma unroll
                    for (int i = 0; i < K3_WALK_CH; i++) y[i] = (uint32_t)tile[(size_t)(r0 + i < R ? r0 + i : R - 1) * TS + sl];
#pragma unroll
                    for (int i = 0; i < K3_WALK_CH; i++) {
                        const int r = r0 + i;
                        if (r < R) {
                            const uint32_t c = y[i] >= P.lower ? y[i] : 0u;
                            if ((mk_tot >> r) & 1u) tot += c;
                            num += c;
                            if ((mk_unit >> r) & 1u) {
                                asm volatile("");
                                const float x = (float)num * __int_as_float(__builtin_amdgcn_readlane(inv_bits, r));
                                m2 = fmaxf(m2, fminf(m1, x));
                                m1 = fmaxf(m1, x);
                                mn = fminf(mn, x);
                                num = 0;
                            }
                            if ((mk_set >> r) & 1u) {
                                asm volatile("");
                                const float thr = fold32 * ((((mk_bi1 >> r) & 1u) ? m2 : mn) + 1e-20f);
                                const bool pass = m1 > thr * (1.0f + 1e-5f);
                                include += pass ? 1 : 0;
                                exact = exact || (!pass && !(m1 < thr * (1.0f - 1e-5f)));
                                m1 = -1.0f; m2 = -1.0f; mn = 3e38f;
                            }
                        }
                    }
                }
                if (live && tot) {
                    if (exact) {
                        queue2[atomicAdd(&s_q2n, 1u)] = (uint16_t)sl;
                    } else if (include >= P.need_hist) {
                        atomicOr(&bmh[sl >> 5], 1u << (sl & 31));
                        nhist++;
                        const double t = (double)tot;
                        if (!(t < P.min_freq || t > P.max_freq)) {
                            atomicOr(&bmr[sl >> 5], 1u << (sl & 31));
                            nrow++;
                        }
                    }
                }
            }
            __syncthreads();
        }
        const uint32_t q2n = s_q2n;
        if (q2n) {
            const int EW = 1 + (R + 3) / 4;
            if (threadIdx.x == 0) {
                s_q3n = 0;
                s_gq0 = (P.gq && q2n) ? atomicAdd(P.gq_n, (unsigned long long)q2n) : ~0ULL;
            }
            __syncthreads();
            const unsigned long long gq0 = s_gq0;
            for (uint32_t q = threadIdx.x; q < q2n; q += F_BLOCK) {
                const int sl = (int)queue2[q];
                const unsigned long long pos = gq0 == ~0ULL ? ~0ULL : gq0 + q;
                if (pos < P.gq_cap) {
                    uint32_t *e = P.gq + pos * EW;
                    e[0] = (uint32_t)(base + sl);
                    for (int r0 = 0; r0 < R; r0 += 4) {
                        uint32_t w = 0;
                        for (int i = 0; i < 4 && r0 + i < R; i++) w |= (uint32_t)tile[(size_t)(r0 + i) * TS + sl] << (8 * i);
                        e[1 + r0 / 4] = w;
                    }
                } else {
                    queue[atomicAdd(&s_q3n, 1u)] = (uint16_t)sl;
                }
            }
            __syncthreads();
            const uint32_t q3n = s_q3n;
            const int wave = threadIdx.x >> 6;
            uint32_t *mine = resolved + (size_t)wave * R;
            for (uint32_t q = wave; q < q3n; q += F_BLOCK / 64) {
                const int sl = (int)queue[q];
                for (int r = lane; r < R; r += 64) {
                    uint32_t y = tile[(size_t)r * TS + sl];
                    if (y == 255u) y = sp_ovf_lookup(l_ovf[r], (int64_t)l_novf[r], (uint32_t)(P.slot_base + base + sl));
                    mine[r] = y >= P.lower ? y : 0u;
                }
                __builtin_amdgcn_wave_barrier();
                __threadfence_block();
                if (lane == 0) {
                    auto cnt_chrom = [&](int c) -> uint32_t { return mine[P.row_of_chrom[c]]; };
                    unsigned long long tot = 0;
                    for (int r = 0; r < R; r++)
                        if (rowdesc[r] & F3_TOT) tot += mine[r];
                    if (tot) {
                        if (!SWAR) nuni++;
                        bool is_row = false, is_hist = false;
                        sp_filter_decide(cnt_chrom, tot, F, is_row, is_hist);
                        if (is_row) { atomicOr(&bmr[sl >> 5], 1u << (sl & 31)); nrow++; }
                        if (is_hist) { atomicOr(&bmh[sl >> 5], 1u << (sl & 31)); nhist++; }
                    }
                }
                __builtin_amdgcn_wave_barrier();
            }
        }
        __syncthreads();
        for (int i = threadIdx.x; i < TS / 64; i += F_BLOCK) {
            const int64_t g = (base >> 6) + i;
            if ((g << 6) < P.nslots) {
                bm_row[g] = (unsigned long long)bmr[2 * i] | ((unsigned long long)bmr[2 * i + 1] << 32);
                bm_hist[g] = (unsigned long long)bmh[2 * i] | ((unsigned long long)bmh[2 * i + 1] << 32);
            }
        }
        __syncthreads();
    }
    unsigned long long t_row = sp_block_sum_u64(nrow, red);
    unsigned long long t_hist = sp_block_sum_u64(nhist, red);
    unsigned long long t_uni = sp_block_sum_u64(nuni, red);
    if (threadIdx.x == 0) {
        blk_row[blockIdx.x] = t_row;
        blk_hist[blockIdx.x] = t_hist;
        if (t_uni) atomicAdd(n_union, t_uni);
    }
}

__global__ void __launch_bounds__(256)
k3_slow(const sp_tabref *__restrict__ tabs, sp_filter_params P, unsigned long long n_entries,
        const int32_t *__restrict__ set_off, const int32_t *__restrict__ unit_off,
        const int32_t *__restrict__ unit_chrom, const double *__restrict__ unit_den,
        unsigned long long *__restrict__ bm_row, unsigned long long *__restrict__ bm_hist,
        unsigned long long *__restrict__ blk_row, unsigned long long *__restrict__ blk_hist,
        unsigned long long *__restrict__ n_union, int count_union) {
    extern __shared__ uint32_t res[];
    const int R = P.R, EW = 1 + (R + 3) / 4, lane = threadIdx.x & 63, wave = threadIdx.x >> 6;
    uint32_t *mine = res + (size_t)wave * R;
    sp_fsets F;
    F.n_sets = P.n_sets;
    F.n_multi = P.n_multi;
    F.baseline = P.baseline;
    F.set_off = set_off;
    F.unit_off = unit_off;
    F.unit_chrom = unit_chrom;
    F.unit_den = unit_den;
    F.unit_inv = unit_den + set_off[P.n_sets];
    F.min_fold = P.min_fold;
    F.min_freq = P.min_freq;
    F.max_freq = P.max_freq;
    F.ratio = P.ratio;
    for (unsigned long long q = (unsigned long long)blockIdx.x * 4 + wave; q < n_entries; q += (unsigned long long)gridDim.x * 4) {
        const uint32_t *e = P.gq + q * EW;
        const uint32_t sl = e[0];
        for (int r = lane; r < R; r += 64) {
            uint32_t y = (e[1 + r / 4] >> (8 * (r & 3))) & 255u;
            if (y == 255u) {
                const sp_tabref t = tabs[P.rowdesc[r] & F3_CHROM_MASK];
                y = sp_ovf_lookup_t(t, (uint32_t)(P.slot_base + sl));
            }
            mine[r] = y >= P.lower ? y : 0u;
        }
        __builtin_amdgcn_wave_barrier();
        __threadfence_block();
        if (lane == 0) {
            auto cnt_chrom = [&](int c) -> uint32_t { return mine[P.row_of_chrom[c]]; };
            unsigned long long tot = 0;
            for (int r = 0; r < R; r++)
                if (P.rowdesc[r] & F3_TOT) tot += mine[r];
            if (tot) {
                if (count_union) atomicAdd(n_union, 1ULL);
                bool is_row = false, is_hist = false;
                sp_filter_decide(cnt_chrom, tot, F, is_row, is_hist);
                if (is_row) {
                    atomicOr(&bm_row[sl >> 6], 1ULL << (sl & 63));
                    atomicAdd(&blk_row[sl / F_SLOTS_PER_BLOCK], 1ULL);
                }
                if (is_hist) {
                    atomicOr(&bm_hist[sl >> 6], 1ULL << (sl & 63));
                    atomicAdd(&blk_hist[sl / F_SLOTS_PER_BLOCK], 1ULL);
                }
            }
        }
        __builtin_amdgcn_wave_barrier();
    }
}

__global__ void scan_excl_u64(unsigned long long *a, int64_t n, unsigned long long *total);

__global__ void __launch_bounds__(F_BLOCK)
k3_emit_slots(int64_t nslots, const unsigned long long *__restrict__ bm, const unsigned long long *__restrict__ blk_off,
              uint32_t *__restrict__ slots) {
    __shared__ unsigned long long wave_cnt[F_WAVES];
    const int lane = threadIdx.x & 63, wave = threadIdx.x >> 6;
    const int64_t blk_base = (int64_t)blockIdx.x * F_SLOTS_PER_BLOCK;
    const int64_t g0 = (blk_base >> 6) + (int64_t)wave * F_GROUPS_PER_WAVE;
    const int64_t ngroups = (nslots + 63) >> 6;
    unsigned long long mycnt = 0;
    for (int g = lane; g < F_GROUPS_PER_WAVE; g += 64)
        if (g0 + g < ngroups) mycnt += __popcll(bm[g0 + g]);
    for (int o = 32; o > 0; o >>= 1) mycnt += __shfl_down(mycnt, o, 64);
    if (lane == 0) wave_cnt[wave] = mycnt;
    __syncthreads();
    unsigned long long off = blk_off[blockIdx.x];
    for (int w = 0; w < wave; w++) off += wave_cnt[w];
    for (int g = 0; g < F_GROUPS_PER_WAVE; g++) {
        if (g0 + g >= ngroups) break;
        const unsigned long long bits = bm[g0 + g];
        if (bits == 0) continue;
        if ((bits >> lane) & 1ULL)
            slots[off + __popcll(bits & ((1ULL << lane) - 1ULL))] = (uint32_t)(((g0 + g) << 6) + lane);
        off += __popcll(bits);
    }
}

__global__ void __launch_bounds__(256)
k3_emit(const sp_tabref *__restrict__ tabs, int C, uint32_t lower, int64_t M, int64_t slot_base, sp_kparams kp,
        const uint32_t *__restrict__ slots, const double *__restrict__ chrom_len,
        unsigned long long *__restrict__ keys, uint32_t *__restrict__ counts,
        double *__restrict__ freqs, unsigned long long *__restrict__ tots) {
    const int64_t r = (int64_t)blockIdx.x * blockDim.x + threadIdx.x;
    if (r >= M) return;
    const int64_t slot = slots[r];
    unsigned long long tot = 0;
    for (int c = 0; c < C; c++) {
        uint32_t v = sp_tab_count(tabs[c], slot, slot_base);
        v = v >= lower ? v : 0u;
        tot += v;
        if (counts) counts[r * C + c] = v;
        if (freqs) freqs[r * C + c] = (double)v / chrom_len[c];
    }
    if (keys) keys[r] = sp_key_of_slot((uint64_t)(slot_base + slot), kp);
    if (tots) tots[r] = tot;
}

static void free_filter_buffers(sp_ctx *ctx) {
    if (ctx->d_flag_row) hipFree(ctx->d_flag_row);
    if (ctx->d_flag_hist) hipFree(ctx->d_flag_hist);
    if (ctx->d_blk_row) hipFree(ctx->d_blk_row);
    if (ctx->d_blk_hist) hipFree(ctx->d_blk_hist);
    ctx->d_flag_row = ctx->d_flag_hist = nullptr;
    ctx->d_blk_row = ctx->d_blk_hist = nullptr;
    ctx->filtered = false;
}


static int filter_C(sp_ctx *ctx) {
    return ctx->sv_on ? (int)ctx->sv_keys.size() : ctx->fv_on ? (int)ctx->fv_tabs.size() : (int)ctx->chroms.size();
}
static sp_tabref filter_tab(sp_ctx *ctx, int i) {
    if (ctx->fv_on) return ctx->fv_tabs[(size_t)i];
    const sp_chrom &c = ctx->chroms[(size_t)i];
    sp_tabref t;
    t.tab = c.d_tab;
    t.ovf = c.d_ovf;
    t.n_ovf = c.n_ovf;
    t.ovf_idx = (c.ovf_idx_n > 0 && c.ovf_idx_n == ((ctx->nslots + (1LL << SP_OVF_SHIFT) - 1) >> SP_OVF_SHIFT) + 1) ? c.d_ovf_idx : nullptr;
    return t;
}
static int64_t filter_len(sp_ctx *ctx, int i) {
    return (ctx->fv_on || ctx->sv_on) ? ctx->fv_lengths[(size_t)i] : ctx->chroms[(size_t)i].length_sum;
}
static int64_t filter_nslots(sp_ctx *ctx) { return ctx->fv_on ? ctx->fv_nslots : ctx->nslots; }
static int64_t filter_base(sp_ctx *ctx) { return ctx->fv_on ? ctx->fv_slot_base : 0; }

static int upload_tabs(sp_ctx *ctx, const sp_tabref **d_tabs, double **d_len) {
    const size_t C = (size_t)filter_C(ctx);
    size_t bytes = C * sizeof(sp_tabref) + C * sizeof(double);
    void *scr = nullptr;
    int rc = sp_scratch(ctx, (int64_t)bytes + 4096, &scr);
    if (rc) return rc;
    std::vector<sp_tabref> h(C);
    std::vector<double> hl(C);
    for (size_t i = 0; i < C; i++) {
        h[i] = filter_tab(ctx, (int)i);
        hl[i] = (double)filter_len(ctx, (int)i);
    }
    SP_HIP(ctx, hipMemcpyAsync(scr, h.data(), C * sizeof(sp_tabref), hipMemcpyHostToDevice, ctx->stream));
    SP_HIP(ctx, hipMemcpyAsync((char *)scr + C * sizeof(sp_tabref), hl.data(), C * sizeof(double),
                              hipMemcpyHostToDevice, ctx->stream));
    SP_HIP(ctx, hipStreamSynchronize(ctx->stream));
    *d_tabs = (const sp_tabref *)scr;
    *d_len = (double *)((char *)scr + C * sizeof(sp_tabref));
    return SP_OK;
}

int sp_sparse_filter(sp_ctx *ctx, int n_sets, const int32_t *set_off, const int32_t *unit_off,
                     const int32_t *unit_chrom, const std::vector<double> &den, double min_fold, int baseline,
                     double min_freq, double max_freq, double ratio);
int sp_sparse_fetch(sp_ctx *ctx, bool hist, uint64_t *keys, uint32_t *counts, double *freqs, uint64_t *tot, bool async);

extern "C" {

int sp_filter_view(sp_ctx *ctx, int C, const void *const *d_tabs, int64_t slot_base, int64_t nslots_view,
                   const int64_t *lengths, int k, int lower_count, const void *const *d_ovf, const int64_t *n_ovf) {
    if (!ctx) return SP_EINVAL;
    if (d_tabs && C > SP_LIST_MAXC)
        return sp_fail(ctx, SP_EUNSUP, "sp_filter_view: a view takes at most %d chromosomes (got %d); more chromosomes are "
                                       "filtered on one GPU", SP_LIST_MAXC, C);
    if (d_tabs && (ctx->sparse_mode || ctx->list_mode)) return sp_fail(ctx, SP_EUNSUP, "sp_filter_view: byte-table engines (k <= 15) only");
    if (!d_tabs) {
        ctx->fv_on = false;
        ctx->fv_tabs.clear();
        ctx->fv_lengths.clear();
        ctx->filtered = false;
        return SP_OK;
    }
    if (C <= 0 || !lengths || slot_base < 0 || nslots_view <= 0 || (slot_base % 64) != 0 || k < 1 || k > 15)
        return sp_fail(ctx, SP_EINVAL, "sp_filter_view: bad arguments (slot_base must be a multiple of 64)");
    ctx->fv_tabs.assign((size_t)C, sp_tabref());
    ctx->fv_lengths.assign((size_t)C, 0);
    for (int i = 0; i < C; i++) {
        if (!d_tabs[i]) return sp_fail(ctx, SP_EINVAL, "sp_filter_view: table %d is NULL", i);
        if ((uintptr_t)d_tabs[i] & 15) return sp_fail(ctx, SP_EINVAL, "sp_filter_view: table %d is not 16-byte aligned", i);
        sp_tabref t;
        t.tab = (const uint8_t *)d_tabs[i];
        t.ovf = (d_ovf && n_ovf && n_ovf[i] > 0) ? (const uint2 *)d_ovf[i] : nullptr;
        t.n_ovf = (d_ovf && n_ovf && n_ovf[i] > 0) ? n_ovf[i] : 0;
        if (t.n_ovf && !t.ovf) return sp_fail(ctx, SP_EINVAL, "sp_filter_view: overflow list %d is NULL", i);
        ctx->fv_tabs[(size_t)i] = t;
        ctx->fv_lengths[(size_t)i] = lengths[i];
    }
    ctx->fv_slot_base = slot_base;
    ctx->fv_nslots = nslots_view;
    ctx->fv_on = true;
    ctx->filtered = false;
    if (ctx->k == 0) {
        ctx->k = k;
        ctx->nslots = sp_dense_slots(k);
    }
    if (ctx->k != k) return sp_fail(ctx, SP_EINVAL, "sp_filter_view: k=%d but the context counted with k=%d", k, ctx->k);
    ctx->lower = lower_count < 1 ? 1 : lower_count;
    return SP_OK;
}

int sp_filter(sp_ctx *ctx, int n_sets, const int32_t *set_off, const int32_t *unit_off,
              const int32_t *unit_chrom, double min_fold, int baseline, double min_freq,
              double max_freq, double ratio, int64_t *n_union, int64_t *n_rows, int64_t *n_hist) {
    if (!ctx || !set_off || !unit_off || !unit_chrom || n_sets <= 0)
        return sp_fail(ctx, SP_EINVAL, "sp_filter: bad arguments");
    if (!ctx->counted && !ctx->fv_on && !ctx->sv_on) return sp_fail(ctx, SP_EINVAL, "sp_filter: call sp_count first");
    SP_HIP(ctx, hipSetDevice(ctx->device));
    if (ctx->copy_stream) SP_HIP(ctx, hipStreamSynchronize(ctx->copy_stream));
    const int C = filter_C(ctx);
    if (min_freq > max_freq)
        return sp_fail(ctx, SP_ESTATE, "`min_freq` (%g) should be lower than `max_freq` (%g)", min_freq,
                       max_freq);
    int n_single = 0, n_units = set_off[n_sets];
    for (int s = 0; s < n_sets; s++) {
        int nu = set_off[s + 1] - set_off[s];
        if (nu == 1) n_single++;
        if (nu > F_MAXU)
            return sp_fail(ctx, SP_EUNSUP, "a homoeologous set has %d subgenome columns; this build supports <= %d",
                           nu, F_MAXU);
        if (nu > 1) {
            int bi = baseline < 0 ? nu + baseline : baseline;
            if (bi < 0 || bi >= nu) return sp_fail(ctx, SP_ESTATE, "list index out of range (baseline=%d)", baseline);
        }
    }
    if (n_single == n_sets) return sp_fail(ctx, SP_ESTATE, "All singletons are not allowed");
    for (int i = 0; i < C; i++)
        if (filter_len(ctx, i) == 0)
            return sp_fail(ctx, SP_ESTATE, "Chromosomes `[%d]` have only 0 kmers", i);
    const int n_uc = unit_off[n_units];
    for (int j = 0; j < n_uc; j++)
        if (unit_chrom[j] < 0 || unit_chrom[j] >= C)
            return sp_fail(ctx, SP_EINVAL, "sp_filter: chromosome index %d out of range", unit_chrom[j]);

    if (ctx->sparse_mode || ctx->list_mode) {
        std::vector<double> den_s((size_t)n_units * 2);
        for (int u = 0; u < n_units; u++) {
            int64_t d = 0;
            for (int j = unit_off[u]; j < unit_off[u + 1]; j++) d += filter_len(ctx, unit_chrom[j]);
            den_s[(size_t)u] = (double)d;
            den_s[(size_t)(n_units + u)] = 1.0 / (double)d;
        }
        int rcs = sp_sparse_filter(ctx, n_sets, set_off, unit_off, unit_chrom, den_s, min_fold, baseline, min_freq,
                                   max_freq, ratio);
        if (rcs) return rcs;
        if (n_union) *n_union = ctx->n_union;
        if (n_rows) *n_rows = ctx->n_rows;
        if (n_hist) *n_hist = ctx->n_hist;
        return SP_OK;
    }
    if (C > SP_LIST_MAXC)
        return sp_fail(ctx, SP_EUNSUP, "sp_filter: byte tables of %d chromosomes: more than %d chromosomes are filtered as "
                                       "lists only -- k = 9..15, a whole-genome count (engine 0 or 3) into library-owned "
                                       "tables on one GPU; no filter view, bound tables or count engines 1 / 2", C, SP_LIST_MAXC);
    const int64_t nslots = filter_nslots(ctx);
    const int64_t nblk = (nslots + F_SLOTS_PER_BLOCK - 1) / F_SLOTS_PER_BLOCK;
    const int64_t ngroups = (nslots + 63) / 64;
    ctx->filtered = false;
    if (!ctx->d_flag_row || ctx->n_fblocks != nblk) {
        free_filter_buffers(ctx);
        SP_HIP(ctx, hipMalloc(&ctx->d_flag_row, (size_t)ngroups * 8));
        SP_HIP(ctx, hipMalloc(&ctx->d_flag_hist, (size_t)ngroups * 8));
        SP_HIP(ctx, hipMalloc(&ctx->d_blk_row, (size_t)(nblk + 1) * 8));
        SP_HIP(ctx, hipMalloc(&ctx->d_blk_hist, (size_t)(nblk + 1) * 8));
    }
    ctx->n_fblocks = nblk;

    std::vector<double> den((size_t)n_units * 2);
    for (int u = 0; u < n_units; u++) {
        int64_t d = 0;
        for (int j = unit_off[u]; j < unit_off[u + 1]; j++) d += filter_len(ctx, unit_chrom[j]);
        den[(size_t)u] = (double)d;
        den[(size_t)(n_units + u)] = 1.0 / (double)d;
    }
    size_t b_set = (size_t)(n_sets + 1) * 4, b_uo = (size_t)(n_units + 1) * 4, b_uc = (size_t)(n_uc > 0 ? n_uc : 1) * 4,
           b_den = (size_t)n_units * 16;
    auto al = [](size_t x) { return (x + 255) & ~(size_t)255; };
    size_t tot_b = al(b_set) + al(b_uo) + al(b_uc) + al(b_den) + al(C * sizeof(sp_tabref)) + 256;
    int rcb = sp_buf_ensure(ctx, ctx->b_fpar, (int64_t)tot_b);
    if (rcb) return rcb;
    char *d_par = (char *)ctx->b_fpar.p;
    char *p = d_par;
    int32_t *d_set = (int32_t *)p; p += al(b_set);
    int32_t *d_uo = (int32_t *)p; p += al(b_uo);
    int32_t *d_uc = (int32_t *)p; p += al(b_uc);
    double *d_den = (double *)p; p += al(b_den);
    sp_tabref *d_tabs = (sp_tabref *)p; p += al(C * sizeof(sp_tabref));
    unsigned long long *d_nuni = (unsigned long long *)p;
    std::vector<sp_tabref> htabs((size_t)C);
    for (int i = 0; i < C; i++) htabs[(size_t)i] = filter_tab(ctx, i);
    hipError_t e = hipSuccess;
    auto cp = [&](void *d, const void *h, size_t n) {
        if (e == hipSuccess && n) e = hipMemcpyAsync(d, h, n, hipMemcpyHostToDevice, ctx->stream);
    };
    cp(d_set, set_off, b_set);
    cp(d_uo, unit_off, b_uo);
    cp(d_uc, unit_chrom, (size_t)n_uc * 4);
    cp(d_den, den.data(), b_den);
    cp(d_tabs, htabs.data(), C * sizeof(sp_tabref));
    if (e == hipSuccess) e = hipMemsetAsync(d_nuni, 0, 32, ctx->stream);
    if (e == hipSuccess) e = hipStreamSynchronize(ctx->stream);
    if (e != hipSuccess)
        return sp_fail(ctx, SP_EHIP, "sp_filter: parameter upload failed: %s", hipGetErrorString(e));
    sp_filter_params P;
    P.C = C;
    P.n_sets = n_sets;
    P.baseline = baseline;
    P.lower = (uint32_t)ctx->lower;
    P.min_fold = min_fold;
    P.min_freq = min_freq;
    P.max_freq = max_freq;
    P.ratio = ratio;
    P.nslots = nslots;
    P.slot_base = filter_base(ctx);
    int TS = F_SLOTS_PER_BLOCK;
    while (TS > SP_TABLE_MIN_TILE && (size_t)C * TS > F_TILE_BYTES) TS >>= 1;
    if ((size_t)C * TS > SP_TABLE_LDS)
        return sp_fail(ctx, SP_EUNSUP, "sp_filter: %d chromosomes exceed the LDS staging budget (at most %d)", C, SP_TABLE_MAXC);
    P.TS = TS;
    P.n_multi = n_sets - n_single;
    P.need_hist = 0;
    while (P.need_hist <= P.n_multi && (double)P.need_hist / (double)P.n_multi < ratio) P.need_hist++;
    P.need_active = (min_fold > 0 && P.n_multi <= 126) ? P.need_hist : 0;
    std::vector<int32_t> rowdesc, row_of_chrom((size_t)C, -1);
    std::vector<float> rowinv;
    P.fast = 1;
    for (int st = 0; st < n_sets; st++) {
        const int nu = set_off[st + 1] - set_off[st];
        if (nu == 1) continue;
        const int bi = baseline < 0 ? nu + baseline : baseline;
        if (!(bi == 1 || bi == nu - 1)) P.fast = 0;
        for (int u = set_off[st]; u < set_off[st + 1]; u++) {
            if (unit_off[u + 1] == unit_off[u]) P.fast = 0;
            for (int j = unit_off[u]; j < unit_off[u + 1]; j++) {
                const int c = unit_chrom[j];
                int d = c;
                if (row_of_chrom[(size_t)c] < 0) {
                    row_of_chrom[(size_t)c] = (int32_t)rowdesc.size();
                    d |= F3_TOT;
                }
                if (j == unit_off[u + 1] - 1) d |= F3_UNIT_END;
                if (j == unit_off[u + 1] - 1 && u == set_off[st + 1] - 1) d |= F3_SET_END;
                if (bi == 1) d |= F3_BI1;
                rowdesc.push_back(d);
                rowinv.push_back((float)den[(size_t)(n_units + u)]);
            }
        }
    }
    P.R_sets = (int)rowdesc.size();
    for (int c = 0; c < C; c++)
        if (row_of_chrom[(size_t)c] < 0) {
            row_of_chrom[(size_t)c] = (int32_t)rowdesc.size();
            rowdesc.push_back(c | F3_TOT);
            rowinv.push_back(0.0f);
        }
    P.R = (int)rowdesc.size();
    if (C > F3_CHROM_MASK) return sp_fail(ctx, SP_EUNSUP, "sp_filter: too many chromosomes");
    TS = F_SLOTS_PER_BLOCK;
    while (TS > SP_TABLE_MIN_TILE && (size_t)P.R * TS > F_TILE_BYTES) TS >>= 1;
    if ((size_t)P.R * TS > SP_TABLE_LDS)
        return sp_fail(ctx, SP_EUNSUP, "sp_filter: %d chromosome rows exceed the LDS staging budget (at most %d)", P.R,
                       SP_TABLE_MAXC);
    P.TS = TS;
    {
        size_t nR = ((size_t)P.R + 7) & ~(size_t)7;
        if (nR < 32) nR = 32;
        std::vector<int32_t> blob(2 * nR + (size_t)C, 0);
        memcpy(blob.data(), rowdesc.data(), (size_t)P.R * 4);
        memcpy(blob.data() + nR, rowinv.data(), (size_t)P.R * 4);
        memcpy(blob.data() + 2 * nR, row_of_chrom.data(), (size_t)C * 4);
        int rcf = sp_buf_ensure(ctx, ctx->b_fflat, (int64_t)blob.size() * 4 + 64);
        if (rcf) return rcf;
        SP_HIP(ctx, hipMemcpyAsync(ctx->b_fflat.p, blob.data(), blob.size() * 4, hipMemcpyHostToDevice, ctx->stream));
        SP_HIP(ctx, hipStreamSynchronize(ctx->stream));
        P.rowdesc = (const int32_t *)ctx->b_fflat.p;
        P.rowinv = (const float *)(P.rowdesc + nR);
        P.row_of_chrom = P.rowdesc + 2 * nR;
    }
    {
        const int EW = 1 + (P.R + 3) / 4;
        unsigned long long cap = (unsigned long long)(nslots / 64 + 4096);
        int rq = sp_buf_ensure(ctx, ctx->b_fq, (int64_t)(cap * EW * 4 + 64));
        if (rq) return rq;
        P.gq = (uint32_t *)((char *)ctx->b_fq.p + 64);
        P.gq_n = (unsigned long long *)ctx->b_fq.p;
        P.gq_cap = cap;
        SP_HIP(ctx, hipMemsetAsync(ctx->b_fq.p, 0, 64, ctx->stream));
    }
    const size_t shmem = (size_t)P.R * TS + (size_t)TS * 4 + (size_t)TS / 4 + (size_t)P.R * 16 + (size_t)P.R * 4 * F_WAVES;
    const bool swar = ctx->lower >= 1 && ctx->lower <= 128;
    const int nch = (swar && P.fast && P.R <= 32) ? 1 : 0;
#define K3_LAUNCH(SW, N)                                                                                          \
    do {                                                                                                          \
        SP_HIP(ctx, hipFuncSetAttribute((const void *)k3_eval<SW, N>, hipFuncAttributeMaxDynamicSharedMemorySize, \
                                        (int)shmem));                                                             \
        SP_LAUNCH(ctx, "k3_eval", (k3_eval<SW, N>), dim3((unsigned)nblk), dim3(F_BLOCK), shmem,                   \
                  (const sp_tabref *)d_tabs, P, d_set, d_uo, d_uc, d_den, (unsigned long long *)ctx->d_flag_row,  \
                  (unsigned long long *)ctx->d_flag_hist, (unsigned long long *)ctx->d_blk_row,                   \
                  (unsigned long long *)ctx->d_blk_hist, d_nuni);                                                 \
    } while (0)
    if (!swar) K3_LAUNCH(false, 0);
    else if (nch == 1) K3_LAUNCH(true, 1);
    else K3_LAUNCH(true, 0);
#undef K3_LAUNCH
    {
        unsigned long long hq = 0;
        SP_HIP(ctx, hipMemcpyAsync(&hq, P.gq_n, 8, hipMemcpyDeviceToHost, ctx->stream));
        SP_HIP(ctx, hipStreamSynchronize(ctx->stream));
        if (hq > P.gq_cap) hq = P.gq_cap;
        if (hq > 0) {
            unsigned long long nb = (hq + 3) / 4;
            if (nb > (unsigned long long)ctx->n_cu * 32) nb = (unsigned long long)ctx->n_cu * 32;
            SP_LAUNCH(ctx, "k3_slow", k3_slow, dim3((unsigned)nb), dim3(256), (size_t)P.R * 16, (const sp_tabref *)d_tabs, P, hq,
                      d_set, d_uo, d_uc, d_den, (unsigned long long *)ctx->d_flag_row, (unsigned long long *)ctx->d_flag_hist,
                      (unsigned long long *)ctx->d_blk_row, (unsigned long long *)ctx->d_blk_hist, d_nuni, swar ? 0 : 1);
        }
    }
    unsigned long long *d_tot = d_nuni + 1;
    SP_LAUNCH(ctx, "scan_excl_u64", scan_excl_u64, dim3(1), dim3(1024), 0,
              (unsigned long long *)ctx->d_blk_row, nblk, d_tot);
    SP_LAUNCH(ctx, "scan_excl_u64", scan_excl_u64, dim3(1), dim3(1024), 0,
              (unsigned long long *)ctx->d_blk_hist, nblk, d_tot + 1);
    unsigned long long h[3] = {0, 0, 0};
    SP_HIP(ctx, hipMemcpyAsync(h, d_tot, 16, hipMemcpyDeviceToHost, ctx->stream));
    SP_HIP(ctx, hipMemcpyAsync(h + 2, d_nuni, 8, hipMemcpyDeviceToHost, ctx->stream));
    SP_HIP(ctx, hipStreamSynchronize(ctx->stream));
    ctx->n_rows = (int64_t)h[0];
    ctx->n_hist = (int64_t)h[1];
    ctx->n_union = (int64_t)h[2];
    ctx->filtered = true;
    if (n_union) *n_union = ctx->n_union;
    if (n_rows) *n_rows = ctx->n_rows;
    if (n_hist) *n_hist = ctx->n_hist;
    return SP_OK;
}

static int emit_common(sp_ctx *ctx, bool hist, uint64_t *keys, uint32_t *counts, double *freqs,
                       uint64_t *tot, int64_t cap, bool async = false) {
    if (!ctx->filtered) return sp_fail(ctx, SP_EINVAL, "call sp_filter first");
    SP_HIP(ctx, hipSetDevice(ctx->device));
    const int64_t M = hist ? ctx->n_hist : ctx->n_rows;
    if (cap < M) return sp_fail(ctx, SP_EINVAL, "capacity %lld < %lld rows", (long long)cap, (long long)M);
    if (M == 0) return SP_OK;
    if (ctx->sparse_mode || ctx->list_mode) return sp_sparse_fetch(ctx, hist, keys, counts, freqs, tot, async);
    const int C = filter_C(ctx);
    const sp_tabref *d_tabs = nullptr;
    double *d_len = nullptr;
    int rc = upload_tabs(ctx, &d_tabs, &d_len);
    if (rc) return rc;
    unsigned long long *d_keys = nullptr, *d_tot = nullptr;
    uint32_t *d_counts = nullptr;
    double *d_freqs = nullptr;
    auto al = [](size_t x) { return (x + 255) & ~(size_t)255; };
    size_t need = (keys ? al((size_t)M * 8) : 0) + (tot ? al((size_t)M * 8) : 0) +
                  (counts ? al((size_t)M * C * 4) : 0) + (freqs ? al((size_t)M * C * 8) : 0);
    rc = sp_buf_ensure(ctx, ctx->b_emit, (int64_t)need);
    if (rc) return rc;
    {
        char *q = (char *)ctx->b_emit.p;
        if (keys) { d_keys = (unsigned long long *)q; q += al((size_t)M * 8); }
        if (tot) { d_tot = (unsigned long long *)q; q += al((size_t)M * 8); }
        if (counts) { d_counts = (uint32_t *)q; q += al((size_t)M * C * 4); }
        if (freqs) { d_freqs = (double *)q; q += al((size_t)M * C * 8); }
    }
    const sp_kparams kp = sp_make_kparams(ctx->k);
    rc = sp_buf_ensure(ctx, ctx->b_slots, M * 4 + 64);
    if (rc) return rc;
    uint32_t *d_slots = (uint32_t *)ctx->b_slots.p;
    SP_LAUNCH(ctx, "k3_emit_slots", k3_emit_slots, dim3((unsigned)ctx->n_fblocks), dim3(F_BLOCK), 0, filter_nslots(ctx),
              (const unsigned long long *)(hist ? ctx->d_flag_hist : ctx->d_flag_row),
              (const unsigned long long *)(hist ? ctx->d_blk_hist : ctx->d_blk_row), d_slots);
    SP_LAUNCH(ctx, hist ? "k3_emit_hist" : "k3_emit", k3_emit, dim3((unsigned)((M + 255) / 256)), dim3(256), 0, d_tabs, C,
              (uint32_t)ctx->lower, M, filter_base(ctx), kp, (const uint32_t *)d_slots, (const double *)d_len, d_keys,
              d_counts, d_freqs, d_tot);
    hipStream_t cs = ctx->stream;
    if (async) {
        if (!ctx->copy_stream) {
            SP_HIP(ctx, hipStreamCreateWithFlags(&ctx->copy_stream, hipStreamNonBlocking));
            SP_HIP(ctx, hipEventCreateWithFlags(&ctx->copy_event, hipEventDisableTiming));
        }
        SP_HIP(ctx, hipEventRecord(ctx->copy_event, ctx->stream));
        SP_HIP(ctx, hipStreamWaitEvent(ctx->copy_stream, ctx->copy_event, 0));
        cs = ctx->copy_stream;
    }
    if (keys) SP_HIP(ctx, hipMemcpyAsync(keys, d_keys, (size_t)M * 8, hipMemcpyDeviceToHost, cs));
    if (tot) SP_HIP(ctx, hipMemcpyAsync(tot, d_tot, (size_t)M * 8, hipMemcpyDeviceToHost, cs));
    if (counts) SP_HIP(ctx, hipMemcpyAsync(counts, d_counts, (size_t)M * C * 4, hipMemcpyDeviceToHost, cs));
    if (freqs) SP_HIP(ctx, hipMemcpyAsync(freqs, d_freqs, (size_t)M * C * 8, hipMemcpyDeviceToHost, cs));
    if (!async) SP_HIP(ctx, hipStreamSynchronize(ctx->stream));
    return SP_OK;
}

int sp_filter_fetch(sp_ctx *ctx, uint64_t *keys, uint32_t *counts, double *freqs, uint64_t *tot,
                    int64_t cap_rows) {
    if (!ctx) return SP_EINVAL;
    return emit_common(ctx, false, keys, counts, freqs, tot, cap_rows);
}

int sp_filter_fetch_async(sp_ctx *ctx, uint64_t *keys, uint32_t *counts, uint64_t *tot, int64_t cap_rows) {
    if (!ctx) return SP_EINVAL;
    return emit_common(ctx, false, keys, counts, nullptr, tot, cap_rows, true);
}

int sp_filter_fetch_wait(sp_ctx *ctx) {
    if (!ctx) return SP_EINVAL;
    if (ctx->copy_stream) SP_HIP(ctx, hipStreamSynchronize(ctx->copy_stream));
    return SP_OK;
}

int sp_filter_fetch_device(sp_ctx *ctx, void *d_keys, void *d_counts, void *d_tot, int64_t cap_rows) {
    if (!ctx) return SP_EINVAL;
    if (!ctx->filtered) return sp_fail(ctx, SP_EINVAL, "call sp_filter first");
    SP_HIP(ctx, hipSetDevice(ctx->device));
    const int64_t M = ctx->n_rows;
    if (cap_rows < M) return sp_fail(ctx, SP_EINVAL, "capacity %lld < %lld rows", (long long)cap_rows, (long long)M);
    if (M == 0) return SP_OK;
    const int C = filter_C(ctx);
    if (ctx->sparse_mode || ctx->list_mode) {
        if (d_keys) SP_HIP(ctx, hipMemcpyAsync(d_keys, ctx->b_sf_keys.p, (size_t)M * 8, hipMemcpyDeviceToDevice, ctx->stream));
        if (d_counts) SP_HIP(ctx, hipMemcpyAsync(d_counts, ctx->b_sf_counts.p, (size_t)M * C * 4, hipMemcpyDeviceToDevice, ctx->stream));
        if (d_tot) SP_HIP(ctx, hipMemcpyAsync(d_tot, ctx->b_sf_tot.p, (size_t)M * 8, hipMemcpyDeviceToDevice, ctx->stream));
        SP_HIP(ctx, hipStreamSynchronize(ctx->stream));
        return SP_OK;
    }
    const sp_tabref *d_tabs = nullptr;
    double *d_len = nullptr;
    int rc = upload_tabs(ctx, &d_tabs, &d_len);
    if (rc) return rc;
    const sp_kparams kp = sp_make_kparams(ctx->k);
    rc = sp_buf_ensure(ctx, ctx->b_slots, M * 4 + 64);
    if (rc) return rc;
    uint32_t *d_slots = (uint32_t *)ctx->b_slots.p;
    SP_LAUNCH(ctx, "k3_emit_slots", k3_emit_slots, dim3((unsigned)ctx->n_fblocks), dim3(F_BLOCK), 0, filter_nslots(ctx),
              (const unsigned long long *)ctx->d_flag_row, (const unsigned long long *)ctx->d_blk_row, d_slots);
    SP_LAUNCH(ctx, "k3_emit", k3_emit, dim3((unsigned)((M + 255) / 256)), dim3(256), 0, d_tabs, C, (uint32_t)ctx->lower, M,
              filter_base(ctx), kp, (const uint32_t *)d_slots, (const double *)d_len, (unsigned long long *)d_keys,
              (uint32_t *)d_counts, (double *)nullptr, (unsigned long long *)d_tot);
    SP_HIP(ctx, hipStreamSynchronize(ctx->stream));
    return SP_OK;
}

int sp_filter_hist(sp_ctx *ctx, uint64_t *tot, int64_t cap) {
    if (!ctx || !tot) return sp_fail(ctx, SP_EINVAL, "sp_filter_hist: bad arguments");
    return emit_common(ctx, true, nullptr, nullptr, nullptr, tot, cap);
}
}
```

Measured before the change: 153.9.

## Stage passing rows during filter and place them from staged buffer at emit

While the filter kernel still holds the count tile in LDS, one wave now writes compact per-row count words for passing slots into a global staging buffer, plus a fast-path bitmap. A new k3_place kernel then emits keys, counts and totals from the staged rows, so the later pass no longer re-probes every chromosome table, and it also replaces the separate slot-list kernel. The parameter upload goes through pinned host memory with a single readback, and k3_slow reads its queue length on the device, which removes a host sync. In exchange the filter kernel does extra work and needs extra memory, and it falls back to the old emit path if the staging buffer overflows.

```diff
diff --git a/include/subphaser_hip.h b/include/subphaser_hip.h
--- a/include/subphaser_hip.h
+++ b/include/subphaser_hip.h
@@ -57,6 +57,7 @@
 int sp_filter_fetch_wait(sp_ctx *ctx);
 int sp_filter_fetch_device(sp_ctx *ctx, void *d_keys, void *d_counts, void *d_tot, int64_t cap_rows);
 int sp_filter_hist(sp_ctx *ctx, uint64_t *tot, int64_t cap);
+int sp_filter_emit_stats(sp_ctx *ctx, int64_t *out);
 
 int sp_labels_set(sp_ctx *ctx, const uint64_t *keys, const uint8_t *sg, int64_t n, int n_sg);
 int sp_labels_set_device(sp_ctx *ctx, const uint64_t *d_keys, const uint8_t *d_sg, int64_t n, int n_sg);
diff --git a/subphaser_amd/_native.py b/subphaser_amd/_native.py
--- a/subphaser_amd/_native.py
+++ b/subphaser_amd/_native.py
@@ -13,7 +13,7 @@
     "sp_version", "sp_last_error", "sp_ctx_create", "sp_ctx_destroy", "sp_sync", "sp_stream",
     "sp_genome_reset", "sp_genome_add", "sp_genome_add_device", "sp_genome_len", "sp_genome_unpack",
     "sp_count", "sp_count_range", "sp_count_recounts", "sp_nslots", "sp_tables_bind", "sp_table_overflow", "sp_table_merge", "sp_table_lengths", "sp_lengths", "sp_dump_size", "sp_dump",
-    "sp_filter_view", "sp_filter", "sp_filter_fetch", "sp_filter_fetch_async", "sp_filter_fetch_wait", "sp_filter_fetch_device", "sp_filter_hist",
+    "sp_filter_view", "sp_filter", "sp_filter_fetch", "sp_filter_fetch_async", "sp_filter_fetch_wait", "sp_filter_fetch_device", "sp_filter_hist", "sp_filter_emit_stats",
     "sp_labels_set", "sp_labels_set_device", "sp_map_nslots", "sp_map_bins", "sp_map_bins_all", "sp_stack_windows", "sp_stack_windows_dev", "sp_stack_enrich", "sp_map_features", "sp_map_intervals", "sp_labels_hit",
     "sp_enrich", "sp_enrich_dev", "sp_kmer_ttest",
     "sp_sparse_sizes", "sp_sparse_sample", "sp_sparse_split", "sp_sparse_export", "sp_sparse_view",
@@ -84,6 +84,7 @@
     L.sp_filter_fetch_async.argtypes = [vp, vp, vp, vp, i64]
     L.sp_filter_fetch_wait.argtypes = [vp]
     L.sp_filter_hist.argtypes = [vp, vp, i64]
+    L.sp_filter_emit_stats.argtypes = [vp, vp]
     L.sp_labels_set.argtypes = [vp, vp, vp, i64, ci]
     L.sp_labels_set_device.argtypes = [vp, vp, vp, i64, ci]
     L.sp_map_nslots.argtypes = [vp, ci, i64, i64, P(i64)]
@@ -545,6 +546,11 @@
         self._ck(self.L.sp_filter_hist(self.h, _p(tot), n_hist))
         return tot
 
+    def filter_emit_stats(self):
+        out = np.zeros(4, np.int64)
+        self._ck(self.L.sp_filter_emit_stats(self.h, _p(out)))
+        return dict(path=int(out[0]), fallbacks=int(out[1]), staged=int(out[2]), slow_rows=int(out[3]))
+
     def labels_set(self, keys, sg, n_sg):
         keys = np.ascontiguousarray(keys, np.uint64)
         sg = np.ascontiguousarray(sg, np.uint8)
diff --git a/subphaser_amd/csrc/sp_common.h b/subphaser_amd/csrc/sp_common.h
--- a/subphaser_amd/csrc/sp_common.h
+++ b/subphaser_amd/csrc/sp_common.h
@@ -158,6 +158,19 @@
     sp_buf b_wtab, b_enr;
     sp_buf b_fq;
     sp_buf b_fflat;
+    sp_buf b_fstage, b_ftile, b_ffast;
+    void *h_fpar = nullptr;
+    int64_t h_fpar_cap = 0;
+    bool st_valid = false;
+    bool st_overflow = false;
+    int st_TS = 0, st_RW = 0;
+    int64_t st_rows = 0;
+    const sp_tabref *st_tabs = nullptr;
+    const double *st_len = nullptr;
+    const int32_t *st_row_of_chrom = nullptr;
+    unsigned long long *st_counters = nullptr;
+    int64_t st_fallbacks = 0;
+    int st_last_path = -1;
     sp_buf b_map, b_mapdesc, b_ival, b_emit, b_fpar, b_win;
     bool map_all_valid = false;
     bool prof = false;
diff --git a/subphaser_amd/csrc/sp_ctx.hip b/subphaser_amd/csrc/sp_ctx.hip
--- a/subphaser_amd/csrc/sp_ctx.hip
+++ b/subphaser_amd/csrc/sp_ctx.hip
@@ -178,6 +178,10 @@
     sp_buf_free(ctx->b_fpar);
     sp_buf_free(ctx->b_fflat);
     sp_buf_free(ctx->b_fq);
+    sp_buf_free(ctx->b_fstage);
+    sp_buf_free(ctx->b_ftile);
+    sp_buf_free(ctx->b_ffast);
+    if (ctx->h_fpar) hipHostFree(ctx->h_fpar);
     sp_buf_free(ctx->b_wtab);
     sp_buf_free(ctx->b_enr);
     sp_buf_free(ctx->b_tt);
diff --git a/subphaser_amd/csrc/sp_filter.hip b/subphaser_amd/csrc/sp_filter.hip
--- a/subphaser_amd/csrc/sp_filter.hip
+++ b/subphaser_amd/csrc/sp_filter.hip
@@ -39,10 +39,82 @@
     uint32_t *gq;
     unsigned long long *gq_n;
     unsigned long long gq_cap;
+    int st_RW;
+    uint32_t *st;
+    uint32_t *st_tile;
+    uint32_t *bm_fast;
+    unsigned long long *st_n;
+    unsigned long long st_cap;
 };
+
+__device__ __forceinline__ uint32_t k3_wave_incl(uint32_t v, int lane) {
+#pragma unroll
+    for (int o = 1; o < 64; o <<= 1) {
+        const uint32_t t = __shfl_up(v, o, 64);
+        if (lane >= o) v += t;
+    }
+    return v;
+}
 
 __device__ __forceinline__ uint32_t k3_ge_mask(uint32_t x, uint32_t addL ) {
     return (((x & 0x7f7f7f7fu) + addL) | x) & 0x80808080u;
+}
+
+__device__ __noinline__ void
+k3_stage_rows(const uint8_t *tile, uint16_t *queue, const uint32_t *bmr, int64_t base, int TS, int R, int lane, int64_t nslots,
+              uint32_t lower, int st_RW, uint32_t *st, uint32_t *st_tile, uint32_t *bm_fast, unsigned long long *st_n,
+              unsigned long long st_cap) {
+    const int NW = TS / 32;
+    const int64_t nwords = ((nslots + 63) >> 6) * 2;
+    uint32_t run = 0;
+#pragma unroll 1
+    for (int i = lane; i < NW; i += 64) {
+        const uint32_t w = bmr[i];
+        if ((base >> 5) + i < nwords) bm_fast[(base >> 5) + i] = w;
+        run += (uint32_t)__popc(w);
+    }
+    run = (uint32_t)__shfl((int)k3_wave_incl(run, lane), 63, 64);
+    if (run) {
+        unsigned long long st0 = 0;
+        if (lane == 0) st0 = atomicAdd(st_n, (unsigned long long)run);
+        uint32_t pos0 = 0;
+#pragma unroll 1
+        for (int i0 = 0; i0 < NW; i0 += 64) {
+            uint32_t bits = i0 + lane < NW ? bmr[i0 + lane] : 0u;
+            const uint32_t c = (uint32_t)__popc(bits), inc = k3_wave_incl(c, lane);
+            uint32_t pos = pos0 + inc - c;
+            while (bits) {
+                queue[pos++] = (uint16_t)(32 * (i0 + lane) + __ffs((int)bits) - 1);
+                bits &= bits - 1;
+            }
+            pos0 += (uint32_t)__shfl((int)inc, 63, 64);
+        }
+        st0 = __shfl(st0, 0, 64);
+        __builtin_amdgcn_wave_barrier();
+        __threadfence_block();
+        if (st0 + run <= st_cap) {
+            const uint32_t RW = (uint32_t)st_RW, sh = 32u - (uint32_t)__clz((int)(RW - 1) | 1);
+            const uint32_t j = lane & ((1u << sh) - 1u);
+            if (lane == 0) st_tile[base >> (__ffs(TS) - 1)] = (uint32_t)st0;
+            uint32_t *__restrict__ dst = st + st0 * RW;
+#pragma unroll 1
+            for (uint32_t row = lane >> sh; row < run; row += 64u >> sh) {
+                if (j < RW) {
+                    const int sl = (int)queue[row];
+                    uint32_t word = 0;
+#pragma unroll
+                    for (int i = 0; i < 4; i++) {
+                        const int r = (int)(4 * j) + i;
+                        const uint32_t y = (uint32_t)tile[(size_t)(r < R ? r : R - 1) * TS + sl];
+                        if (r < R && y >= lower) word |= y << (8 * i);
+                    }
+                    dst[row * RW + j] = word;
+                }
+            }
+        } else if (lane == 0) {
+            st_n[1] = 1ULL;
+        }
+    }
 }
 
 #ifndef K3_STAGE
@@ -318,6 +390,9 @@
                 }
             }
             __syncthreads();
+            if (P.st_RW && threadIdx.x < 64)
+                k3_stage_rows(tile, queue, bmr, base, TS, R, lane, P.nslots, P.lower, P.st_RW, P.st, P.st_tile, P.bm_fast,
+                              P.st_n, P.st_cap);
         }
         const uint32_t q2n = s_q2n;
         if (q2n) {
@@ -393,7 +468,7 @@
 }
 
 __global__ void __launch_bounds__(256)
-k3_slow(const sp_tabref *__restrict__ tabs, sp_filter_params P, unsigned long long n_entries,
+k3_slow(const sp_tabref *__restrict__ tabs, sp_filter_params P,
         const int32_t *__restrict__ set_off, const int32_t *__restrict__ unit_off,
         const int32_t *__restrict__ unit_chrom, const double *__restrict__ unit_den,
         unsigned long long *__restrict__ bm_row, unsigned long long *__restrict__ bm_hist,
@@ -415,6 +490,8 @@
     F.min_freq = P.min_freq;
     F.max_freq = P.max_freq;
     F.ratio = P.ratio;
+    unsigned long long n_entries = *P.gq_n;
+    if (n_entries > P.gq_cap) n_entries = P.gq_cap;
     for (unsigned long long q = (unsigned long long)blockIdx.x * 4 + wave; q < n_entries; q += (unsigned long long)gridDim.x * 4) {
         const uint32_t *e = P.gq + q * EW;
         const uint32_t sl = e[0];
@@ -499,6 +576,93 @@
     if (tots) tots[r] = tot;
 }
 
+#define K3_PLACE_CH 1024
+static_assert(F_SLOTS_PER_BLOCK == 64 * F_BLOCK, "k3_place: one thread per 64-slot group of a filter block");
+__global__ void __launch_bounds__(F_BLOCK)
+k3_place(const sp_tabref *__restrict__ tabs, int C, uint32_t lower, int64_t nslots, int64_t slot_base, sp_kparams kp, int TS,
+         int RW, const unsigned long long *__restrict__ bm_row, const unsigned long long *__restrict__ bm_fast,
+         const unsigned long long *__restrict__ blk_off, const uint32_t *__restrict__ st_tile,
+         const uint32_t *__restrict__ st, const int32_t *__restrict__ row_of_chrom, const double *__restrict__ chrom_len,
+         unsigned long long *__restrict__ keys, uint32_t *__restrict__ counts, double *__restrict__ freqs,
+         unsigned long long *__restrict__ tots, unsigned long long *__restrict__ n_slow) {
+    __shared__ uint32_t s_fast[F_BLOCK], s_wfin[F_WAVES], s_wfast[F_WAVES];
+    __shared__ uint32_t l_slot[K3_PLACE_CH], l_src[K3_PLACE_CH];
+    const int t = threadIdx.x, lane = t & 63, wave = t >> 6;
+    const int64_t g = (int64_t)blockIdx.x * F_BLOCK + t, ngroups = (nslots + 63) >> 6;
+    const unsigned long long fin = g < ngroups ? bm_row[g] : 0ULL, fast = g < ngroups ? bm_fast[g] & fin : 0ULL;
+    const uint32_t cf = (uint32_t)__popcll(fin), cs = (uint32_t)__popcll(fast);
+    uint32_t xf = k3_wave_incl(cf, lane), xs = k3_wave_incl(cs, lane);
+    if (lane == 63) { s_wfin[wave] = xf; s_wfast[wave] = xs; }
+    __syncthreads();
+    uint32_t n_blk = 0;
+    for (int w = 0; w < F_WAVES; w++) {
+        if (w < wave) { xf += s_wfin[w]; xs += s_wfast[w]; }
+        n_blk += s_wfin[w];
+    }
+    if (n_blk == 0) return;
+    xf -= cf; xs -= cs;
+    s_fast[t] = xs;
+    __syncthreads();
+    const int GT = TS / 64;
+    const uint32_t src0 = cs ? st_tile[g / GT] + (xs - s_fast[t & ~(GT - 1)]) : 0u;
+    const unsigned long long off0 = blk_off[blockIdx.x];
+    uint32_t my_slow = 0;
+    for (uint32_t c0 = 0; c0 < n_blk; c0 += K3_PLACE_CH) {
+        if (xf < c0 + K3_PLACE_CH && xf + cf > c0) {
+            unsigned long long bits = fin;
+            uint32_t pos = xf, src = src0;
+            while (bits) {
+                const int b = __ffsll((long long)bits) - 1;
+                const bool staged = (fast >> b) & 1ULL;
+                if (pos >= c0 && pos < c0 + K3_PLACE_CH) {
+                    l_slot[pos - c0] = (uint32_t)(g * 64 + b);
+                    l_src[pos - c0] = staged ? src : 0xffffffffu;
+                    if (!staged) my_slow++;
+                }
+                src += staged ? 1u : 0u;
+                pos++;
+                bits &= bits - 1;
+            }
+        }
+        __syncthreads();
+        const uint32_t nrow = n_blk - c0 < K3_PLACE_CH ? n_blk - c0 : K3_PLACE_CH;
+        const unsigned long long out0 = off0 + c0;
+        if (counts || freqs)
+            for (uint32_t idx = t; idx < nrow * (uint32_t)C; idx += F_BLOCK) {
+                const uint32_t r = idx / (uint32_t)C, c = idx - r * (uint32_t)C, src = l_src[r];
+                uint32_t v;
+                if (src != 0xffffffffu) {
+                    v = reinterpret_cast<const uint8_t *>(st + (size_t)src * RW)[row_of_chrom[c]];
+                } else {
+                    v = sp_tab_count(tabs[c], (int64_t)l_slot[r], slot_base);
+                    v = v >= lower ? v : 0u;
+                }
+                if (counts) counts[out0 * C + idx] = v;
+                if (freqs) freqs[out0 * C + idx] = (double)v / chrom_len[c];
+            }
+        for (uint32_t r = t; r < nrow; r += F_BLOCK) {
+            const uint32_t src = l_src[r];
+            if (keys) keys[out0 + r] = sp_key_of_slot((uint64_t)(slot_base + (int64_t)l_slot[r]), kp);
+            if (tots) {
+                unsigned long long tot = 0;
+                for (int c = 0; c < C; c++) {
+                    uint32_t v;
+                    if (src != 0xffffffffu) {
+                        v = reinterpret_cast<const uint8_t *>(st + (size_t)src * RW)[row_of_chrom[c]];
+                    } else {
+                        v = sp_tab_count(tabs[c], (int64_t)l_slot[r], slot_base);
+                        v = v >= lower ? v : 0u;
+                    }
+                    tot += v;
+                }
+                tots[out0 + r] = tot;
+            }
+        }
+        __syncthreads();
+    }
+    if (my_slow) atomicAdd(n_slow, (unsigned long long)my_slow);
+}
+
 static void free_filter_buffers(sp_ctx *ctx) {
     if (ctx->d_flag_row) hipFree(ctx->d_flag_row);
     if (ctx->d_flag_hist) hipFree(ctx->d_flag_hist);
@@ -672,35 +836,6 @@
         den[(size_t)u] = (double)d;
         den[(size_t)(n_units + u)] = 1.0 / (double)d;
     }
-    size_t b_set = (size_t)(n_sets + 1) * 4, b_uo = (size_t)(n_units + 1) * 4, b_uc = (size_t)(n_uc > 0 ? n_uc : 1) * 4,
-           b_den = (size_t)n_units * 16;
-    auto al = [](size_t x) { return (x + 255) & ~(size_t)255; };
-    size_t tot_b = al(b_set) + al(b_uo) + al(b_uc) + al(b_den) + al(C * sizeof(sp_tabref)) + 256;
-    int rcb = sp_buf_ensure(ctx, ctx->b_fpar, (int64_t)tot_b);
-    if (rcb) return rcb;
-    char *d_par = (char *)ctx->b_fpar.p;
-    char *p = d_par;
-    int32_t *d_set = (int32_t *)p; p += al(b_set);
-    int32_t *d_uo = (int32_t *)p; p += al(b_uo);
-    int32_t *d_uc = (int32_t *)p; p += al(b_uc);
-    double *d_den = (double *)p; p += al(b_den);
-    sp_tabref *d_tabs = (sp_tabref *)p; p += al(C * sizeof(sp_tabref));
-    unsigned long long *d_nuni = (unsigned long long *)p;
-    std::vector<sp_tabref> htabs((size_t)C);
-    for (int i = 0; i < C; i++) htabs[(size_t)i] = filter_tab(ctx, i);
-    hipError_t e = hipSuccess;
-    auto cp = [&](void *d, const void *h, size_t n) {
-        if (e == hipSuccess && n) e = hipMemcpyAsync(d, h, n, hipMemcpyHostToDevice, ctx->stream);
-    };
-    cp(d_set, set_off, b_set);
-    cp(d_uo, unit_off, b_uo);
-    cp(d_uc, unit_chrom, (size_t)n_uc * 4);
-    cp(d_den, den.data(), b_den);
-    cp(d_tabs, htabs.data(), C * sizeof(sp_tabref));
-    if (e == hipSuccess) e = hipMemsetAsync(d_nuni, 0, 32, ctx->stream);
-    if (e == hipSuccess) e = hipStreamSynchronize(ctx->stream);
-    if (e != hipSuccess)
-        return sp_fail(ctx, SP_EHIP, "sp_filter: parameter upload failed: %s", hipGetErrorString(e));
     sp_filter_params P;
     P.C = C;
     P.n_sets = n_sets;
@@ -712,11 +847,6 @@
     P.ratio = ratio;
     P.nslots = nslots;
     P.slot_base = filter_base(ctx);
-    int TS = F_SLOTS_PER_BLOCK;
-    while (TS > SP_TABLE_MIN_TILE && (size_t)C * TS > F_TILE_BYTES) TS >>= 1;
-    if ((size_t)C * TS > SP_TABLE_LDS)
-        return sp_fail(ctx, SP_EUNSUP, "sp_filter: %d chromosomes exceed the LDS staging budget (at most %d)", C, SP_TABLE_MAXC);
-    P.TS = TS;
     P.n_multi = n_sets - n_single;
     P.need_hist = 0;
     while (P.need_hist <= P.n_multi && (double)P.need_hist / (double)P.n_multi < ratio) P.need_hist++;
@@ -755,40 +885,89 @@
         }
     P.R = (int)rowdesc.size();
     if (C > F3_CHROM_MASK) return sp_fail(ctx, SP_EUNSUP, "sp_filter: too many chromosomes");
-    TS = F_SLOTS_PER_BLOCK;
+    int TS = F_SLOTS_PER_BLOCK;
     while (TS > SP_TABLE_MIN_TILE && (size_t)P.R * TS > F_TILE_BYTES) TS >>= 1;
     if ((size_t)P.R * TS > SP_TABLE_LDS)
         return sp_fail(ctx, SP_EUNSUP, "sp_filter: %d chromosome rows exceed the LDS staging budget (at most %d)", P.R,
                        SP_TABLE_MAXC);
     P.TS = TS;
+    size_t nR = ((size_t)P.R + 7) & ~(size_t)7;
+    if (nR < 32) nR = 32;
+    const size_t b_set = (size_t)(n_sets + 1) * 4, b_uo = (size_t)(n_units + 1) * 4, b_uc = (size_t)(n_uc > 0 ? n_uc : 1) * 4,
+                 b_den = (size_t)n_units * 16, b_flat = (2 * nR + (size_t)C) * 4;
+    auto al = [](size_t x) { return (x + 255) & ~(size_t)255; };
+    const size_t o_set = 0, o_uo = o_set + al(b_set), o_uc = o_uo + al(b_uo), o_den = o_uc + al(b_uc), o_tabs = o_den + al(b_den),
+                 o_len = o_tabs + al(C * sizeof(sp_tabref)), o_cnt = o_len + al((size_t)C * 8), tot_b = o_cnt + 256;
+    if (ctx->h_fpar_cap < (int64_t)(tot_b + b_flat)) {
+        if (ctx->h_fpar) hipHostFree(ctx->h_fpar);
+        ctx->h_fpar = nullptr;
+        ctx->h_fpar_cap = 0;
+        SP_HIP(ctx, hipHostMalloc(&ctx->h_fpar, 2 * (tot_b + b_flat), hipHostMallocDefault));
+        ctx->h_fpar_cap = (int64_t)(2 * (tot_b + b_flat));
+    }
+    int rcb = sp_buf_ensure(ctx, ctx->b_fpar, (int64_t)tot_b);
+    if (rcb) return rcb;
+    rcb = sp_buf_ensure(ctx, ctx->b_fflat, (int64_t)b_flat + 64);
+    if (rcb) return rcb;
+    char *h_par = (char *)ctx->h_fpar, *d_par = (char *)ctx->b_fpar.p;
+    memset(h_par, 0, tot_b + b_flat);
+    memcpy(h_par + o_set, set_off, b_set);
+    memcpy(h_par + o_uo, unit_off, b_uo);
+    memcpy(h_par + o_uc, unit_chrom, (size_t)n_uc * 4);
+    memcpy(h_par + o_den, den.data(), b_den);
+    for (int i = 0; i < C; i++) {
+        reinterpret_cast<sp_tabref *>(h_par + o_tabs)[i] = filter_tab(ctx, i);
+        reinterpret_cast<double *>(h_par + o_len)[i] = (double)filter_len(ctx, i);
+    }
     {
-        size_t nR = ((size_t)P.R + 7) & ~(size_t)7;
-        if (nR < 32) nR = 32;
-        std::vector<int32_t> blob(2 * nR + (size_t)C, 0);
-        memcpy(blob.data(), rowdesc.data(), (size_t)P.R * 4);
-        memcpy(blob.data() + nR, rowinv.data(), (size_t)P.R * 4);
-        memcpy(blob.data() + 2 * nR, row_of_chrom.data(), (size_t)C * 4);
-        int rcf = sp_buf_ensure(ctx, ctx->b_fflat, (int64_t)blob.size() * 4 + 64);
-        if (rcf) return rcf;
-        SP_HIP(ctx, hipMemcpyAsync(ctx->b_fflat.p, blob.data(), blob.size() * 4, hipMemcpyHostToDevice, ctx->stream));
-        SP_HIP(ctx, hipStreamSynchronize(ctx->stream));
-        P.rowdesc = (const int32_t *)ctx->b_fflat.p;
-        P.rowinv = (const float *)(P.rowdesc + nR);
-        P.row_of_chrom = P.rowdesc + 2 * nR;
-    }
+        int32_t *flat = reinterpret_cast<int32_t *>(h_par + tot_b);
+        memcpy(flat, rowdesc.data(), (size_t)P.R * 4);
+        memcpy(flat + nR, rowinv.data(), (size_t)P.R * 4);
+        memcpy(flat + 2 * nR, row_of_chrom.data(), (size_t)C * 4);
+    }
+    int32_t *d_set = (int32_t *)(d_par + o_set), *d_uo = (int32_t *)(d_par + o_uo), *d_uc = (int32_t *)(d_par + o_uc);
+    double *d_den = (double *)(d_par + o_den);
+    sp_tabref *d_tabs = (sp_tabref *)(d_par + o_tabs);
+    unsigned long long *d_nuni = (unsigned long long *)(d_par + o_cnt);
+    P.rowdesc = (const int32_t *)ctx->b_fflat.p;
+    P.rowinv = (const float *)(P.rowdesc + nR);
+    P.row_of_chrom = P.rowdesc + 2 * nR;
     {
         const int EW = 1 + (P.R + 3) / 4;
         unsigned long long cap = (unsigned long long)(nslots / 64 + 4096);
         int rq = sp_buf_ensure(ctx, ctx->b_fq, (int64_t)(cap * EW * 4 + 64));
         if (rq) return rq;
-        P.gq = (uint32_t *)((char *)ctx->b_fq.p + 64);
-        P.gq_n = (unsigned long long *)ctx->b_fq.p;
+        P.gq = (uint32_t *)ctx->b_fq.p;
+        P.gq_n = d_nuni + 6;
         P.gq_cap = cap;
-        SP_HIP(ctx, hipMemsetAsync(ctx->b_fq.p, 0, 64, ctx->stream));
-    }
-    const size_t shmem = (size_t)P.R * TS + (size_t)TS * 4 + (size_t)TS / 4 + (size_t)P.R * 16 + (size_t)P.R * 4 * F_WAVES;
+    }
     const bool swar = ctx->lower >= 1 && ctx->lower <= 128;
     const int nch = (swar && P.fast && P.R <= 32) ? 1 : 0;
+    const char *env_emit = getenv("SP_FILTER_EMIT"), *env_cap = getenv("SP_FILTER_STAGE_CAP");
+    const bool stage = nch == 1 && !(env_emit && !strcmp(env_emit, "gather"));
+    P.st_RW = 0;
+    P.st = P.st_tile = P.bm_fast = nullptr;
+    P.st_n = d_nuni + 3;
+    P.st_cap = 0;
+    ctx->st_valid = ctx->st_overflow = false;
+    if (stage) {
+        P.st_RW = (P.R + 3) / 4;
+        P.st_cap = (unsigned long long)(nslots / 64 + 4096);
+        if (env_cap) {
+            const long long v = atoll(env_cap);
+            if (v < (long long)P.st_cap) P.st_cap = (unsigned long long)(v > 0 ? v : 0);
+        }
+        int rs = sp_buf_ensure(ctx, ctx->b_fstage, (int64_t)(P.st_cap * P.st_RW * 4 + 64));
+        if (!rs) rs = sp_buf_ensure(ctx, ctx->b_ftile, ((nslots + TS - 1) / TS) * 4 + 64);
+        if (!rs) rs = sp_buf_ensure(ctx, ctx->b_ffast, ngroups * 8);
+        if (rs) return rs;
+        P.st = (uint32_t *)ctx->b_fstage.p;
+        P.st_tile = (uint32_t *)ctx->b_ftile.p;
+        P.bm_fast = (uint32_t *)ctx->b_ffast.p;
+    }
+    SP_HIP(ctx, hipMemcpyAsync(d_par, h_par, tot_b, hipMemcpyHostToDevice, ctx->stream));
+    SP_HIP(ctx, hipMemcpyAsync(ctx->b_fflat.p, h_par + tot_b, b_flat, hipMemcpyHostToDevice, ctx->stream));
+    const size_t shmem = (size_t)P.R * TS + (size_t)TS * 4 + (size_t)TS / 4 + (size_t)P.R * 16 + (size_t)P.R * 4 * F_WAVES;
 #define K3_LAUNCH(SW, N)                                                                                          \
     do {                                                                                                          \
         SP_HIP(ctx, hipFuncSetAttribute((const void *)k3_eval<SW, N>, hipFuncAttributeMaxDynamicSharedMemorySize, \
@@ -802,35 +981,63 @@
     else if (nch == 1) K3_LAUNCH(true, 1);
     else K3_LAUNCH(true, 0);
 #undef K3_LAUNCH
-    {
-        unsigned long long hq = 0;
-        SP_HIP(ctx, hipMemcpyAsync(&hq, P.gq_n, 8, hipMemcpyDeviceToHost, ctx->stream));
-        SP_HIP(ctx, hipStreamSynchronize(ctx->stream));
-        if (hq > P.gq_cap) hq = P.gq_cap;
-        if (hq > 0) {
-            unsigned long long nb = (hq + 3) / 4;
-            if (nb > (unsigned long long)ctx->n_cu * 32) nb = (unsigned long long)ctx->n_cu * 32;
-            SP_LAUNCH(ctx, "k3_slow", k3_slow, dim3((unsigned)nb), dim3(256), (size_t)P.R * 16, (const sp_tabref *)d_tabs, P, hq,
-                      d_set, d_uo, d_uc, d_den, (unsigned long long *)ctx->d_flag_row, (unsigned long long *)ctx->d_flag_hist,
-                      (unsigned long long *)ctx->d_blk_row, (unsigned long long *)ctx->d_blk_hist, d_nuni, swar ? 0 : 1);
-        }
-    }
+    SP_LAUNCH(ctx, "k3_slow", k3_slow, dim3((unsigned)ctx->n_cu * 32), dim3(256), (size_t)P.R * 16, (const sp_tabref *)d_tabs, P,
+              d_set, d_uo, d_uc, d_den, (unsigned long long *)ctx->d_flag_row, (unsigned long long *)ctx->d_flag_hist,
+              (unsigned long long *)ctx->d_blk_row, (unsigned long long *)ctx->d_blk_hist, d_nuni, swar ? 0 : 1);
     unsigned long long *d_tot = d_nuni + 1;
     SP_LAUNCH(ctx, "scan_excl_u64", scan_excl_u64, dim3(1), dim3(1024), 0,
               (unsigned long long *)ctx->d_blk_row, nblk, d_tot);
     SP_LAUNCH(ctx, "scan_excl_u64", scan_excl_u64, dim3(1), dim3(1024), 0,
               (unsigned long long *)ctx->d_blk_hist, nblk, d_tot + 1);
-    unsigned long long h[3] = {0, 0, 0};
-    SP_HIP(ctx, hipMemcpyAsync(h, d_tot, 16, hipMemcpyDeviceToHost, ctx->stream));
-    SP_HIP(ctx, hipMemcpyAsync(h + 2, d_nuni, 8, hipMemcpyDeviceToHost, ctx->stream));
+    unsigned long long h[5] = {0, 0, 0, 0, 0};
+    SP_HIP(ctx, hipMemcpyAsync(h, d_nuni, sizeof(h), hipMemcpyDeviceToHost, ctx->stream));
     SP_HIP(ctx, hipStreamSynchronize(ctx->stream));
-    ctx->n_rows = (int64_t)h[0];
-    ctx->n_hist = (int64_t)h[1];
-    ctx->n_union = (int64_t)h[2];
+    ctx->n_union = (int64_t)h[0];
+    ctx->n_rows = (int64_t)h[1];
+    ctx->n_hist = (int64_t)h[2];
     ctx->filtered = true;
+    ctx->st_valid = stage && h[4] == 0;
+    ctx->st_overflow = stage && h[4] != 0;
+    ctx->st_rows = (int64_t)h[3];
+    ctx->st_TS = TS;
+    ctx->st_RW = P.st_RW;
+    ctx->st_tabs = d_tabs;
+    ctx->st_len = (const double *)(d_par + o_len);
+    ctx->st_row_of_chrom = P.row_of_chrom;
+    ctx->st_counters = d_nuni;
     if (n_union) *n_union = ctx->n_union;
     if (n_rows) *n_rows = ctx->n_rows;
     if (n_hist) *n_hist = ctx->n_hist;
+    return SP_OK;
+}
+
+static int emit_rows(sp_ctx *ctx, unsigned long long *d_keys, uint32_t *d_counts, double *d_freqs, unsigned long long *d_tot) {
+    const int C = filter_C(ctx);
+    const int64_t M = ctx->n_rows;
+    const sp_kparams kp = sp_make_kparams(ctx->k);
+    ctx->st_last_path = ctx->st_valid ? 1 : 0;
+    if (ctx->st_valid) {
+        SP_HIP(ctx, hipMemsetAsync(ctx->st_counters + 5, 0, 8, ctx->stream));
+        SP_LAUNCH(ctx, "k3_place", k3_place, dim3((unsigned)ctx->n_fblocks), dim3(F_BLOCK), 0, ctx->st_tabs, C,
+                  (uint32_t)ctx->lower, filter_nslots(ctx), filter_base(ctx), kp, ctx->st_TS, ctx->st_RW,
+                  (const unsigned long long *)ctx->d_flag_row, (const unsigned long long *)ctx->b_ffast.p,
+                  (const unsigned long long *)ctx->d_blk_row, (const uint32_t *)ctx->b_ftile.p,
+                  (const uint32_t *)ctx->b_fstage.p, ctx->st_row_of_chrom, ctx->st_len, d_keys, d_counts, d_freqs, d_tot,
+                  ctx->st_counters + 5);
+        return SP_OK;
+    }
+    if (ctx->st_overflow) ctx->st_fallbacks++;
+    const sp_tabref *d_tabs = nullptr;
+    double *d_len = nullptr;
+    int rc = upload_tabs(ctx, &d_tabs, &d_len);
+    if (rc) return rc;
+    rc = sp_buf_ensure(ctx, ctx->b_slots, M * 4 + 64);
+    if (rc) return rc;
+    uint32_t *d_slots = (uint32_t *)ctx->b_slots.p;
+    SP_LAUNCH(ctx, "k3_emit_slots", k3_emit_slots, dim3((unsigned)ctx->n_fblocks), dim3(F_BLOCK), 0, filter_nslots(ctx),
+              (const unsigned long long *)ctx->d_flag_row, (const unsigned long long *)ctx->d_blk_row, d_slots);
+    SP_LAUNCH(ctx, "k3_emit", k3_emit, dim3((unsigned)((M + 255) / 256)), dim3(256), 0, d_tabs, C, (uint32_t)ctx->lower, M,
+              filter_base(ctx), kp, (const uint32_t *)d_slots, (const double *)d_len, d_keys, d_counts, d_freqs, d_tot);
     return SP_OK;
 }
 
@@ -843,10 +1050,7 @@
     if (M == 0) return SP_OK;
     if (ctx->sparse_mode || ctx->list_mode) return sp_sparse_fetch(ctx, hist, keys, counts, freqs, tot, async);
     const int C = filter_C(ctx);
-    const sp_tabref *d_tabs = nullptr;
-    double *d_len = nullptr;
-    int rc = upload_tabs(ctx, &d_tabs, &d_len);
-    if (rc) return rc;
+    int rc = SP_OK;
     unsigned long long *d_keys = nullptr, *d_tot = nullptr;
     uint32_t *d_counts = nullptr;
     double *d_freqs = nullptr;
@@ -862,16 +1066,24 @@
         if (counts) { d_counts = (uint32_t *)q; q += al((size_t)M * C * 4); }
         if (freqs) { d_freqs = (double *)q; q += al((size_t)M * C * 8); }
     }
-    const sp_kparams kp = sp_make_kparams(ctx->k);
-    rc = sp_buf_ensure(ctx, ctx->b_slots, M * 4 + 64);
-    if (rc) return rc;
-    uint32_t *d_slots = (uint32_t *)ctx->b_slots.p;
-    SP_LAUNCH(ctx, "k3_emit_slots", k3_emit_slots, dim3((unsigned)ctx->n_fblocks), dim3(F_BLOCK), 0, filter_nslots(ctx),
-              (const unsigned long long *)(hist ? ctx->d_flag_hist : ctx->d_flag_row),
-              (const unsigned long long *)(hist ? ctx->d_blk_hist : ctx->d_blk_row), d_slots);
-    SP_LAUNCH(ctx, hist ? "k3_emit_hist" : "k3_emit", k3_emit, dim3((unsigned)((M + 255) / 256)), dim3(256), 0, d_tabs, C,
-              (uint32_t)ctx->lower, M, filter_base(ctx), kp, (const uint32_t *)d_slots, (const double *)d_len, d_keys,
-              d_counts, d_freqs, d_tot);
+    if (!hist) {
+        rc = emit_rows(ctx, d_keys, d_counts, d_freqs, d_tot);
+        if (rc) return rc;
+    } else {
+        const sp_kparams kp = sp_make_kparams(ctx->k);
+        const sp_tabref *d_tabs = nullptr;
+        double *d_len = nullptr;
+        rc = upload_tabs(ctx, &d_tabs, &d_len);
+        if (rc) return rc;
+        rc = sp_buf_ensure(ctx, ctx->b_slots, M * 4 + 64);
+        if (rc) return rc;
+        uint32_t *d_slots = (uint32_t *)ctx->b_slots.p;
+        SP_LAUNCH(ctx, "k3_emit_slots", k3_emit_slots, dim3((unsigned)ctx->n_fblocks), dim3(F_BLOCK), 0, filter_nslots(ctx),
+                  (const unsigned long long *)ctx->d_flag_hist, (const unsigned long long *)ctx->d_blk_hist, d_slots);
+        SP_LAUNCH(ctx, "k3_emit_hist", k3_emit, dim3((unsigned)((M + 255) / 256)), dim3(256), 0, d_tabs, C,
+                  (uint32_t)ctx->lower, M, filter_base(ctx), kp, (const uint32_t *)d_slots, (const double *)d_len, d_keys,
+                  d_counts, d_freqs, d_tot);
+    }
     hipStream_t cs = ctx->stream;
     if (async) {
         if (!ctx->copy_stream) {
@@ -922,20 +1134,25 @@
         SP_HIP(ctx, hipStreamSynchronize(ctx->stream));
         return SP_OK;
     }
-    const sp_tabref *d_tabs = nullptr;
-    double *d_len = nullptr;
-    int rc = upload_tabs(ctx, &d_tabs, &d_len);
+    int rc = emit_rows(ctx, (unsigned long long *)d_keys, (uint32_t *)d_counts, nullptr, (unsigned long long *)d_tot);
     if (rc) return rc;
-    const sp_kparams kp = sp_make_kparams(ctx->k);
-    rc = sp_buf_ensure(ctx, ctx->b_slots, M * 4 + 64);
-    if (rc) return rc;
-    uint32_t *d_slots = (uint32_t *)ctx->b_slots.p;
-    SP_LAUNCH(ctx, "k3_emit_slots", k3_emit_slots, dim3((unsigned)ctx->n_fblocks), dim3(F_BLOCK), 0, filter_nslots(ctx),
-              (const unsigned long long *)ctx->d_flag_row, (const unsigned long long *)ctx->d_blk_row, d_slots);
-    SP_LAUNCH(ctx, "k3_emit", k3_emit, dim3((unsigned)((M + 255) / 256)), dim3(256), 0, d_tabs, C, (uint32_t)ctx->lower, M,
-              filter_base(ctx), kp, (const uint32_t *)d_slots, (const double *)d_len, (unsigned long long *)d_keys,
-              (uint32_t *)d_counts, (double *)nullptr, (unsigned long long *)d_tot);
     SP_HIP(ctx, hipStreamSynchronize(ctx->stream));
+    return SP_OK;
+}
+
+int sp_filter_emit_stats(sp_ctx *ctx, int64_t *out) {
+    if (!ctx || !out) return sp_fail(ctx, SP_EINVAL, "sp_filter_emit_stats: bad arguments");
+    out[0] = ctx->st_last_path;
+    out[1] = ctx->st_fallbacks;
+    out[2] = ctx->st_rows;
+    out[3] = 0;
+    if (ctx->st_last_path == 1) {
+        unsigned long long h = 0;
+        SP_HIP(ctx, hipSetDevice(ctx->device));
+        SP_HIP(ctx, hipMemcpyAsync(&h, ctx->st_counters + 5, 8, hipMemcpyDeviceToHost, ctx->stream));
+        SP_HIP(ctx, hipStreamSynchronize(ctx->stream));
+        out[3] = (int64_t)h;
+    }
     return SP_OK;
 }
 
```

Result: slower. 144.3 (-6.2%).
